# apache/datafusion

Measured on AMD Instinct MI355X. Metric: tpch_q3_hash_join_rows_per_sec, higher is better.
Workload: dtype int64 keys / decimal128 payload; 1 GPU; INNER hash-join orders⋈lineitem on o_orderkey, TPC-H SF100, Q3 payload (o_orderdate,o_shippriority,l_orderkey,l_extendedprice,l_discount), device-resident inputs; build_rows=150000000, probe_rows=599960064, output_rows=599960064, join_table=rank_map, probe=single_pass_unordered, parallelism=single GPU, exchange=none

## Files before the change

datafusion_amd/csrc/aggregate.hip:

```cpp
#include <algorithm>
#include <cstdio>
#include <cstdlib>

#include "device.hpp"
#include "internal.hpp"
#include "rowprog_host.hpp"
#include "grouped.hpp"

namespace dfgpu {

void pack_bytes_to_bitmap(const uint8_t* bytes, int64_t n, uint64_t* words);

constexpr int MAX_AGGS = 16;
constexpr uint32_t PROBE_LIMIT = 256;

enum AccKind : int { ACC_SUM_I64 = 0, ACC_SUM_I128 = 1, ACC_SUM_F64 = 2, ACC_MIN_I64 = 3, ACC_MAX_I64 = 4, ACC_COUNT = 5, ACC_COUNT_STAR = 6,
                     ACC_AND = 7, ACC_OR = 8, ACC_XOR = 9, ACC_KIND_COUNT = 10 };
struct AccKindText {
  const char* type;
  const char* from_u64[2];
  const char* to_u64[2];
  const char* neutral;
  const char* atomic;
  const char* cell_cast;
// ... 1641 lines not shown
      InternCtx sc = ictx;
      sc.slots = sslots->as<uint32_t>();
      sc.mask = 2 * SAMPLE - 1;
      {
        ProfileScope ps("agg_intern_sample", key_bytes / total * SAMPLE);
        k_intern_claim<<<grid_for(SAMPLE, BLOCK), BLOCK, 0, r.stream>>>(sc, SAMPLE, flag->as<int>(), nullptr, 0);
        k_count_slots<<<grid_for(2 * SAMPLE, BLOCK), BLOCK, 0, r.stream>>>(sc.slots, (uint64_t)(2 * SAMPLE), (uint32_t)(SAMPLE / 4), cnt->as<unsigned long long>());
        DFGPU_HIP(hipGetLastError());
      }
      unsigned long long c2[2] = {0, 0};
      d2h(c2, cnt->ptr, 16);
      DFGPU_HIP(hipMemsetAsync(flag->ptr, 0, 4, r.stream));
      const double d_all = (double)c2[0], d_early = (double)c2[1];
      const double est = d_all < 1.25 * d_early ? 2.0 * d_all : d_all / (double)SAMPLE * (double)total;
      uint64_t want = 1 << 16;
      while ((double)want < 3.0 * est && want < cap_max) want <<= 1;
      cap = std::max<uint64_t>(cap, want);
    }
  }
  if (cap > cap_max && !direct_n) cap = cap_max;
  while (!direct_n) {
    R.slots = make_zero_buf((cap + 1) * 4);
    ictx.slots = R.slots->as<uint32_t>();
    ictx.mask = cap - 1;
    if (keyed) {
      R.keyed = make_buf((cap + 1) * sizeof(KeyedSlot));
      ictx.keyed = R.keyed->as<KeyedSlot>();
      k_keyed_clear<<<grid_for((int64_t)cap + 1, BLOCK), BLOCK, 0, r.stream>>>(ictx.keyed, cap + 1);
    }
    if (total) {
      ProfileScope ps(keyed ? "agg_intern_claim_keyed" : "agg_intern_claim", key_bytes);
      if (want_row_slots && !R.row_slot) R.row_slot = make_buf((size_t)total * 4);
      uint32_t* rs = R.row_slot ? R.row_slot->as<uint32_t>() : nullptr;
      if (keyed) {
        k_intern_claim_keyed<<<grid_for((total + KEYED_ROWS - 1) / KEYED_ROWS, BLOCK), BLOCK, 0, r.stream>>>(ictx, total, flag->as<int>(), row_mask, G0, rs);
        k_keyed_rows<<<grid_for((int64_t)cap + 1, BLOCK), BLOCK, 0, r.stream>>>(ictx.keyed, cap + 1, ictx.slots);
      }
      else k_intern_claim<<<grid_for(total, BLOCK), BLOCK, 0, r.stream>>>(ictx, total, flag->as<int>(), row_mask, G0, rs);
      DFGPU_HIP(hipGetLastError());
    }
    int ovf = 0;
    d2h(&ovf, flag->ptr, 4);
    if (!ovf) break;
    DFGPU_CHECK(cap < cap_max, "group table overflow at maximum capacity");
    cap = std::min<uint64_t>(cap_max, cap * 16);
    DFGPU_HIP(hipMemsetAsync(flag->ptr, 0, 4, r.stream));
  }
  A.capacity_hint = (int64_t)cap;
  const int64_t n_words = (total + 63) / 64;
  BufPtr rep_mask = make_zero_buf((size_t)(n_words ? n_words : 1) * 8);
  BufPtr prefix = make_buf((size_t)(n_words + 1) * 8);
  const uint64_t n_slots = cap + (keyed ? 1 : 0);
  k_mark_reps<<<grid_for((int64_t)n_slots, BLOCK), BLOCK, 0, r.stream>>>(R.slots->as<uint32_t>(), n_slots, rep_mask->as<unsigned long long>());
  scan_mask_popcounts(rep_mask->as<uint64_t>(), nullptr, total, prefix->as<uint64_t>());
  R.G1 = (int64_t)read_u64(prefix->as<uint64_t>() + n_words);
  R.slot_gid = make_buf((cap + 1) * 4);
  BufPtr rep_row = make_buf((size_t)(R.G1 ? R.G1 : 1) * 8);
  k_slot_gids<<<grid_for((int64_t)n_slots, BLOCK), BLOCK, 0, r.stream>>>(R.slots->as<uint32_t>(), n_slots, rep_mask->as<uint64_t>(), prefix->as<uint64_t>(),
                                                                      R.slot_gid->as<uint32_t>(), rep_row->as<int64_t>());
  DFGPU_HIP(hipGetLastError());
  Table gk;
  gk.nrows = R.G1;
  for (int g = 0; g < ngk; g++) gk.cols.push_back(gather_column(R.cat_keys[g], rep_row->as<int64_t>(), R.G1, false));
  A.group_keys = std::move(gk);
  return R;
}

__global__ __launch_bounds__(BLOCK) void k_split128(const unsigned long long* __restrict__ cells, int64_t n, unsigned long long* __restrict__ lo, unsigned long long* __restrict__ hi) {
  for (int64_t i = (int64_t)blockIdx.x * BLOCK + threadIdx.x; i < n; i += (int64_t)gridDim.x * BLOCK) {
    lo[i] = cells[2 * i];
    hi[i] = cells[2 * i + 1];
  }
}
static void materialize_seen(Aggregate& A, int64_t G) {
  for (AggState& a : A.aggs) {
    if (!a.seen_all) continue;
    if (G > 0 && a.seen) DFGPU_HIP(hipMemsetD32Async((hipDeviceptr_t)a.seen->ptr, 1, (size_t)G, rt().stream));
    a.seen_all = false;
  }
}
static void split_interleaved(Aggregate& A, int64_t G) {
  materialize_seen(A, G);
  for (AggState& a : A.aggs) {
    if (!a.inter) continue;
    if (G > 0) {
      k_split128<<<grid_for(G, BLOCK), BLOCK, 0, rt().stream>>>(a.inter->as<unsigned long long>(), G, a.lo->as<unsigned long long>(), a.hi->as<unsigned long long>());
      DFGPU_HIP(hipGetLastError());
    }
    a.inter.reset();
  }
}

constexpr int FM_MAX = 4 * MAX_AGGS;
struct FillMany {
  void* p[FM_MAX];
  unsigned long long v[FM_MAX];
  int elem[FM_MAX];
};
__global__ __launch_bounds__(BLOCK) void k_fill_many(FillMany f, int64_t n) {
  const int c = blockIdx.y;
  for (int64_t i = (int64_t)blockIdx.x * BLOCK + threadIdx.x; i < n; i += (int64_t)gridDim.x * BLOCK) {
    if (f.elem[c] == 8) reinterpret_cast<unsigned long long*>(f.p[c])[i] = f.v[c];
    else reinterpret_cast<uint32_t*>(f.p[c])[i] = (uint32_t)f.v[c];
  }
}
static std::vector<AccPlan> grow_accumulators(Aggregate& A, int64_t G0, int64_t G1, bool init = true) {
  std::vector<AccPlan> plans;
  const bool final_mode = A.final_mode();
// ... 1451 lines not shown
        hmm[0] = cached->min;
        hmm[1] = cached->max;
        range_known = true;
      }
    }
  }
  if (range_known) {
    hflags[0] = 0;
    hflags[1] = 1;
  } else {
    {
      ProfileScope ps("agg_dense_key_range", key_bytes);
      jit_launch(f_minmax, grid, BLOCK, 0, &args, sizeof(args));
    }
    d2h(hmm, mm->ptr, 16);
    d2h(hflags, flags->ptr, 8);
  }
  const bool any_rows = hflags[1] != 0, null_group = hflags[0] != 0;
  uint64_t range = any_rows ? (uint64_t)hmm[1] - (uint64_t)hmm[0] + 1 : 0;
  if (range > (1ull << 36) || range > (uint64_t)n * 64) return false;
  fix_argument_types(A, cp, arg_out);
  const int64_t n_words = (int64_t)((range + 63) / 64) + 1;
  BufPtr bits = make_zero_buf((size_t)n_words * 8);
  BufPtr prefix = make_buf((size_t)(n_words + 1) * 8);
  args.bits = bits->as<unsigned long long>();
  args.kmin = any_rows ? hmm[0] : 0;
  const int ncw = (int)cell_kind.size();
  PartValues pv;
  pv.want_rep_mask = option_on("agg.gather_emit", true);
  const bool by_parts = any_rows && !null_group && dense_accumulate_partitioned(A, in, pred, accs, acc_col, acc_val, acc_agg, ncw, args.kmin, range, pv);
  auto dense_emit_of = [&]() {
    DenseEmit e{};
    for (const Ent& en : entries) {
      AggState& a = A.aggs[(size_t)en.agg];
      if (en.is_avg_count) {
        e.dst[e.n_dst] = a.cnt->as<unsigned long long>();
        e.src_word[e.n_dst++] = en.cell;
      } else {
        e.dst[e.n_dst] = a.lo->as<unsigned long long>();
        e.src_word[e.n_dst++] = en.cell;
        if (en.kind == ACC_SUM_I128) {
          e.dst[e.n_dst] = a.hi->as<unsigned long long>();
          e.src_word[e.n_dst++] = en.cell + 1;
        }
        e.seen_dst[e.n_seen] = a.seen->as<uint32_t>();
        e.seen_bit[e.n_seen++] = en.seen_bit;
      }
    }
    return e;
  };
  if (by_parts && pv.rep_mask) {
    const int64_t row_words = (n + 63) / 64;
    BufPtr rprefix = make_buf((size_t)(row_words + 1) * 8);
    scan_mask_popcounts(pv.rep_mask->as<uint64_t>(), nullptr, n, rprefix->as<uint64_t>());
    const int64_t G = (int64_t)read_u64(rprefix->as<uint64_t>() + row_words);
    grow_accumulators(A, 0, G, false);
    const DenseEmit e = dense_emit_of();
    int kci = -1;
    DFGPU_CHECK(is_plain_column(A.group_nodes[0], A.group_roots[0], &kci) && kci >= 0 && kci < (int)in.cols.size(), "internal: the partitioned node's key is not a column");
    const Column& kin = in.cols[(size_t)kci];
    Column kc = alloc_column(kf, A.group_names[0], G);
    kc.dict = kin.dict;
    if (G) {
      ProfileScope ps("agg_dense_gather_emit", n * type_width(kf.type) + G * (type_width(kf.type) + 16 * (int64_t)e.n_dst + 4 * (int64_t)e.n_seen));
      const int g = (int)std::min<int64_t>((row_words + GE_TILE_WORDS - 1) / GE_TILE_WORDS, 2048);
      const uint64_t* rm = pv.rep_mask->as<uint64_t>();
      const uint64_t* rp = rprefix->as<uint64_t>();
      const unsigned long long* cv = pv.cells_v->as<unsigned long long>();
      switch (type_width(kf.type)) {
        case 8: k_dense_gather_emit<int64_t><<<g, BLOCK, 0, r.stream>>>(rm, rp, row_words, (const int64_t*)kin.ptr(), args.kmin, cv, std::max(1, ncw), e, (int64_t*)kc.data->ptr); break;
        case 1: k_dense_gather_emit<uint8_t><<<g, BLOCK, 0, r.stream>>>(rm, rp, row_words, (const uint8_t*)kin.ptr(), args.kmin, cv, std::max(1, ncw), e, (uint8_t*)kc.data->ptr); break;
        default:
          if (kf.type == DFGPU_UINT32) k_dense_gather_emit<uint32_t><<<g, BLOCK, 0, r.stream>>>(rm, rp, row_words, (const uint32_t*)kin.ptr(), args.kmin, cv, std::max(1, ncw), e, (uint32_t*)kc.data->ptr);
          else k_dense_gather_emit<int32_t><<<g, BLOCK, 0, r.stream>>>(rm, rp, row_words, (const int32_t*)kin.ptr(), args.kmin, cv, std::max(1, ncw), e, (int32_t*)kc.data->ptr);
          break;
      }
      DFGPU_HIP(hipGetLastError());
    }
    Table gk;
    gk.nrows = G;
    gk.cols.push_back(std::move(kc));
    A.group_keys = std::move(gk);
    A.ngroups = G;
    DFGPU_HIP(hipStreamSynchronize(r.stream));
    return true;
  }
  if (by_parts) {
    k_presence_bits<<<grid_for(n_words, BLOCK / WAVE), BLOCK, 0, r.stream>>>(pv.first_row_v->as<uint32_t>(), range, n_words, bits->as<uint64_t>());
    DFGPU_HIP(hipGetLastError());
  } else if (any_rows) {
    ProfileScope ps("agg_dense_setbits", key_bytes);
    jit_launch(f_setbits, grid, BLOCK, 0, &args, sizeof(args));
  }
  scan_mask_popcounts(bits->as<uint64_t>(), nullptr, n_words * 64, prefix->as<uint64_t>());
  const int64_t Gk = (int64_t)read_u64(prefix->as<uint64_t>() + n_words);
  const int64_t G = Gk + (null_group ? 1 : 0);
  BufPtr first_row = make_buf((size_t)std::max<int64_t>(G, 1) * 4);
  BufPtr seen = by_parts ? make_buf((size_t)std::max<int64_t>(G, 1) * 4) : make_zero_buf((size_t)std::max<int64_t>(G, 1) * 4);
  BufPtr cells = make_buf((size_t)std::max(1, ncw) * std::max<int64_t>(G, 1) * 8);
  args.prefix = prefix->as<uint64_t>();
  args.first_row = first_row->as<uint32_t>();
  args.cells = cells->as<unsigned long long>();
  args.seen = seen->as<uint32_t>();
  args.G = G;
  args.null_group = null_group ? Gk : -1;
  if (by_parts) {
    if (G) {
      ProfileScope ps("agg_dense_values_to_groups", (int64_t)range * (4 + 8 * ncw) + G * (8 + 8 * ncw));
      k_values_to_groups<<<grid_for((int64_t)range, BLOCK), BLOCK, 0, r.stream>>>(bits->as<uint64_t>(), prefix->as<uint64_t>(), pv.first_row_v->as<uint32_t>(),
                                                                                 pv.cells_v->as<unsigned long long>(), pv.vstride, range, ncw, G, first_row->as<uint32_t>(),
                                                                                 cells->as<unsigned long long>(), seen->as<uint32_t>(), (uint32_t)((1ull << accs.size()) - 1ull));
      DFGPU_HIP(hipGetLastError());
    }
  } else {
    DFGPU_HIP(hipMemsetAsync(first_row->ptr, 0xFF, (size_t)std::max<int64_t>(G, 1) * 4, r.stream));
    for (int w = 0; w < ncw && G; w++)
      k_fill_u64<<<grid_for(G, BLOCK), BLOCK, 0, r.stream>>>(acc_identity(cell_kind[(size_t)w]), G, cells->as<unsigned long long>() + (int64_t)w * G);
    if (G) {
      ProfileScope ps("agg_dense_accumulate", n * cp.input_bytes_per_row);
      jit_launch(f_acc, grid, BLOCK, 0, &args, sizeof(args));
    }
  }
  const int64_t row_words = (n + 63) / 64;
  BufPtr rep_mask = make_zero_buf((size_t)row_words * 8);
  BufPtr rprefix = make_buf((size_t)(row_words + 1) * 8);
  if (G) k_mark_first_rows<<<grid_for(G, BLOCK), BLOCK, 0, r.stream>>>(first_row->as<uint32_t>(), G, rep_mask->as<unsigned long long>());
  scan_mask_popcounts(rep_mask->as<uint64_t>(), nullptr, n, rprefix->as<uint64_t>());
  DFGPU_CHECK((int64_t)read_u64(rprefix->as<uint64_t>() + row_words) == G, "dense-key node: first-row marks do not match the group count");
  grow_accumulators(A, 0, G, false);
  const DenseEmit e = dense_emit_of();
  BufPtr new_gid = make_buf((size_t)std::max<int64_t>(G, 1) * 4);
  BufPtr key_i64 = make_zero_buf((size_t)std::max<int64_t>(G, 1) * 8);
  if (G) {
    ProfileScope ps("agg_dense_emit", G * (4 + 8 * (int64_t)e.n_dst));
    k_dense_permute<<<grid_for(G, BLOCK), BLOCK, 0, r.stream>>>(first_row->as<uint32_t>(), cells->as<unsigned long long>(), seen->as<uint32_t>(), G,
                                                                rep_mask->as<uint64_t>(), rprefix->as<uint64_t>(), new_gid->as<uint32_t>(), e);
    k_dense_keys<<<grid_for(n_words, BLOCK / WAVE), BLOCK, 0, r.stream>>>(bits->as<uint64_t>(), prefix->as<uint64_t>(), n_words, args.kmin, new_gid->as<uint32_t>(),
                                                                          key_i64->as<unsigned long long>());
    DFGPU_HIP(hipGetLastError());
  }
  Column kc = alloc_column(kf, A.group_names[0], G);
  {
    int key_col = -1;
    if (is_plain_column(A.group_nodes[0], A.group_roots[0], &key_col) && key_col >= 0 && key_col < (int)in.cols.size()) kc.dict = in.cols[key_col].dict;
  }
  if (G) {
    int mode = 0;
    if (kf.type == DFGPU_INT32 || kf.type == DFGPU_DATE32 || kf.type == DFGPU_UINT32) mode = 3;
    else if (kf.type == DFGPU_UINT8) mode = 4;
    k_emit_values<<<grid_for(G, BLOCK), BLOCK, 0, r.stream>>>(mode, key_i64->as<unsigned long long>(), nullptr, nullptr, G, kc.data->ptr, nullptr);
    DFGPU_HIP(hipGetLastError());
    if (null_group) {
      uint32_t ng = 0;
      d2h(&ng, new_gid->as<uint32_t>() + Gk, 4);
      std::vector<uint8_t> vb((size_t)G, 1);
      vb[ng] = 0;
      BufPtr dvb = make_buf((size_t)G + 64);
      h2d_async(dvb->ptr, vb.data(), (size_t)G);
      kc.validity = make_buf(bitmap_bytes(G));
      pack_bytes_to_bitmap(dvb->as<uint8_t>(), G, kc.validity->as<uint64_t>());
      kc.null_count = 1;
      DFGPU_HIP(hipStreamSynchronize(r.stream));
    }
  }
  Table gk;
  gk.nrows = G;
  gk.cols.push_back(std::move(kc));
  A.group_keys = std::move(gk);
  A.ngroups = G;
  DFGPU_HIP(hipStreamSynchronize(r.stream));
  return true;
}

template <typename T>
__global__ __launch_bounds__(BLOCK) void k_run_heads(const T* __restrict__ key, int64_t n, uint64_t* __restrict__ heads) {
  const int64_t n_words = (n + 63) >> 6;
  const int64_t wave = ((int64_t)blockIdx.x * BLOCK + threadIdx.x) >> 6;
  const int64_t n_waves = ((int64_t)gridDim.x * BLOCK) >> 6;
  const unsigned lane = lane_id();
  constexpr int U = 4;
  for (int64_t w0 = wave * U; w0 < n_words; w0 += n_waves * U) {
// ... 248 lines not shown
  src += "  }\n}\n";
  return src + args_size_check(sizeof(RunsNodeArgs), "RunsNodeArgs");
}

static bool agg_update_sorted_runs_jit(Aggregate& A, const Table& in, const dfgpu_expr* pred) {
  Runtime& r = rt();
  const int64_t n = in.nrows;
  if (pred || !option_on("jit", true) || !option_on("agg.runs", true) || A.group_roots.empty() || A.ngroups != 0) return false;
  if (n < option_int("jit.min_rows", policy().rows_worth_a_pass()) || n >= 0xFFFFFFFFll) return false;
  int key_col = -1;
  if (!is_plain_column(A.group_nodes[0], A.group_roots[0], &key_col) || key_col < 0 || key_col >= (int)in.cols.size()) return false;
  const Column& kcol = in.cols[(size_t)key_col];
  const dfgpu_field kf = kcol.field;
  if (kcol.validity || !(kf.type == DFGPU_INT32 || kf.type == DFGPU_INT64 || kf.type == DFGPU_DATE32 || kf.type == DFGPU_UINT32 || kf.type == DFGPU_UINT8)) return false;
  std::vector<int> more_keys;
  for (size_t g = 1; g < A.group_roots.size(); g++) {
    int c = -1;
    if (!is_plain_column(A.group_nodes[g], A.group_roots[g], &c) || c < 0 || c >= (int)in.cols.size()) return false;
    const Column& mc = in.cols[(size_t)c];
    if (mc.validity || mc.field.type == DFGPU_BOOL || mc.field.type == DFGPU_UTF8) return false;
    more_keys.push_back(c);
  }
  if (!column_stats(const_cast<Column&>(kcol), n).nondecreasing) return false;
  std::string why;
  RowProgramCompiler comp(in);
  dfgpu_expr ke{A.group_nodes[0].data(), (int)A.group_nodes[0].size(), A.group_roots[0]};
  const int key_out = comp.add_output(ke);
  const std::vector<int> arg_out = compile_agg_arguments(comp, A);
  CompiledProgram cp;
  if (!comp.finish(cp, why)) return false;
  const std::vector<AccEntry> entries = accumulator_entries(A, cp, arg_out);
  std::vector<RunsAcc> accs;
  for (const AccEntry& en : entries) {
    const dfgpu_field& t = en.type;
    accs.push_back({en.kind, en.val, en.kind == ACC_SUM_I128 && t.type == DFGPU_DECIMAL128 && t.precision > 0 && t.precision <= 16,
                    en.kind == ACC_SUM_I128 && A.aggs[(size_t)en.agg].func == DFGPU_AGG_SUM && t.type == DFGPU_DECIMAL128});
  }
  if (accs.size() > (size_t)RUNS_MAX_ACCS) return false;
  const std::string source = agg_runs_node_source(cp, cp.src_out_vals[(size_t)key_out], kf.type, accs);
  hipFunction_t f_acc = nullptr;
  if (!jit_get_kernels(source, {{"runs_accumulate", &f_acc}})) return false;
  const int64_t n_words = (n + 63) / 64;
  BufPtr heads = make_buf((size_t)n_words * 8);
  {
    ProfileScope ps("agg_runs_heads", n * type_width(kf.type));
    const int g = grid_for(n_words, (BLOCK / WAVE) * 4);
    switch (type_width(kf.type)) {
      case 8: k_run_heads<uint64_t><<<g, BLOCK, 0, r.stream>>>((const uint64_t*)kcol.ptr(), n, heads->as<uint64_t>()); break;
      case 4: k_run_heads<uint32_t><<<g, BLOCK, 0, r.stream>>>((const uint32_t*)kcol.ptr(), n, heads->as<uint64_t>()); break;
      default: k_run_heads<uint8_t><<<g, BLOCK, 0, r.stream>>>((const uint8_t*)kcol.ptr(), n, heads->as<uint64_t>()); break;
    }
    DFGPU_HIP(hipGetLastError());
  }
  BufPtr prefix = make_buf((size_t)(n_words + 1) * 8);
  scan_mask_popcounts(heads->as<uint64_t>(), nullptr, n, prefix->as<uint64_t>());
  BufPtr long_flag = make_zero_buf(8);
  k_run_long_flag<<<grid_for(n_words, BLOCK), BLOCK, 0, r.stream>>>(heads->as<uint64_t>(), n_words, long_flag->as<uint32_t>());
  if (!more_keys.empty()) {
    int64_t bytes = 0;
    for (int c : more_keys) bytes += n * type_width(in.cols[(size_t)c].field.type);
    ProfileScope ps("agg_runs_dependent_keys", bytes);
    const int g = grid_for(n, BLOCK * 4);
    for (int c : more_keys) {
      const Column& mc = in.cols[(size_t)c];
      uint32_t* fl = long_flag->as<uint32_t>() + 1;
      switch (type_width(mc.field.type)) {
        case 16: k_run_dependent<uint4><<<g, BLOCK, 0, r.stream>>>((const uint4*)mc.ptr(), heads->as<uint64_t>(), n, fl); break;
        case 8: k_run_dependent<uint64_t><<<g, BLOCK, 0, r.stream>>>((const uint64_t*)mc.ptr(), heads->as<uint64_t>(), n, fl); break;
        case 4: k_run_dependent<uint32_t><<<g, BLOCK, 0, r.stream>>>((const uint32_t*)mc.ptr(), heads->as<uint64_t>(), n, fl); break;
        default: k_run_dependent<uint8_t><<<g, BLOCK, 0, r.stream>>>((const uint8_t*)mc.ptr(), heads->as<uint64_t>(), n, fl); break;
      }
    }
    DFGPU_HIP(hipGetLastError());
  }
  const int64_t G = (int64_t)read_u64(prefix->as<uint64_t>() + n_words);
  uint32_t flags[2] = {0, 0};
  d2h(flags, long_flag->ptr, 8);
  if (flags[1]) return false;
  const uint32_t has_long = flags[0];
  fix_argument_types(A, cp, arg_out);
  grow_accumulators(A, 0, G, has_long != 0);
  Column kc = alloc_like(kcol, G);
  kc.name = A.group_names[0];
  RunsNodeArgs args{};
  set_input_columns(args, cp);
  args.heads = heads->as<uint64_t>();
  args.prefix = prefix->as<uint64_t>();
  args.key_out = kc.data->ptr;
  args.n = n;
  for (size_t e = 0; e < entries.size(); e++) {
    AggState& a = A.aggs[(size_t)entries[e].agg];
    if (entries[e].is_avg_count) {
      args.cell[2 * e] = a.cnt->as<unsigned long long>();
    } else if (accs[e].inter) {
      a.inter = has_long ? make_zero_buf((size_t)(G ? G : 1) * 16) : make_buf((size_t)(G ? G : 1) * 16);
      args.cell[2 * e] = a.inter->as<unsigned long long>();
      args.cell[2 * e + 1] = a.inter->as<unsigned long long>() + 1;
      args.seen[e] = a.seen->as<uint32_t>();
    } else {
      args.cell[2 * e] = a.lo->as<unsigned long long>();
      if (entries[e].kind == ACC_SUM_I128) args.cell[2 * e + 1] = a.hi->as<unsigned long long>();
      args.seen[e] = a.seen->as<uint32_t>();
    }
    if (!entries[e].is_avg_count && accs[e].val >= 0 && !cp.src_maybe_null[(size_t)accs[e].val] && option_on("agg.runs_seen_all", true)) {
      args.seen[e] = nullptr;
      a.seen_all = true;
    }
  }
  {
    ProfileScope ps("agg_runs_accumulate", n * cp.input_bytes_per_row);
    const int max_blocks = (int)option_int("agg.runs_max_blocks", 1 << 30);
    jit_launch(f_acc, std::max(1, std::min(grid_for(n_words, BLOCK / WAVE), max_blocks)), BLOCK, 0, &args, sizeof(args));
  }
  Table gk;
  gk.nrows = G;
  gk.cols.push_back(std::move(kc));
  if (!more_keys.empty()) {
    Table heads_rows = compact_table(in, more_keys, heads->as<uint64_t>(), nullptr);
    for (size_t g = 0; g < more_keys.size(); g++) {
      heads_rows.cols[g].name = A.group_names[g + 1];
      gk.cols.push_back(std::move(heads_rows.cols[g]));
    }
  }
  A.group_keys = std::move(gk);
  A.ngroups = G;
  DFGPU_HIP(hipStreamSynchronize(r.stream));
  return true;
}

__global__ __launch_bounds__(BLOCK) void k_small_reset(SmallAccSet accs, int D, uint32_t* __restrict__ g_first, uint32_t* __restrict__ g_seen) {
// ... 1038 lines not shown
```

datafusion_amd/csrc/device.hpp:

```cpp
#pragma once
#include <hip/hip_runtime.h>
#include <stdint.h>

namespace dfgpu {

typedef __int128 i128;
typedef unsigned __int128 u128;

constexpr int WAVE = 64;
constexpr int BLOCK = 256;

__device__ __forceinline__ unsigned lane_id() { return threadIdx.x & 63u; }

#ifndef DFGPU_STREAM_NT
#define DFGPU_STREAM_NT 3
#endif
template <typename T>
__device__ __forceinline__ T stream_load(const T* p) {
#if DFGPU_STREAM_NT & 1
  return __builtin_nontemporal_load(p);
#else
  return *p;
#endif
}
// ... 156 lines not shown
__device__ __forceinline__ bool keys_equal(const KeySet& a, int64_t ia, const KeySet& b, int64_t ib, bool null_equals_null) {
  for (int c = 0; c < a.n; c++) {
    bool va = !a.c[c].valid || bit_at(a.c[c].valid, ia);
    bool vb = !b.c[c].valid || bit_at(b.c[c].valid, ib);
    if (!va || !vb) {
      if (null_equals_null && !va && !vb) continue;
      return false;
    }
    uint64_t alo, ahi, blo, bhi;
    load_words(a.c[c], ia, alo, ahi);
    load_words(b.c[c], ib, blo, bhi);
    if (alo != blo || ahi != bhi) return false;
  }
  return true;
}

__host__ __device__ __forceinline__ int32_t date32_part(int32_t days, int part) {
  const int64_t z = (int64_t)days + 719468;
  const int64_t era = (z >= 0 ? z : z - 146096) / 146097;
  const int64_t doe = z - era * 146097;
  const int64_t yoe = (doe - doe / 1460 + doe / 36524 - doe / 146096) / 365;
  const int64_t doy = doe - (365 * yoe + yoe / 4 - yoe / 100);
  const int64_t mp = (5 * doy + 2) / 153;
  const int64_t d = doy - (153 * mp + 2) / 5 + 1;
  const int64_t m = mp < 10 ? mp + 3 : mp - 9;
  const int64_t y = yoe + era * 400 + (m <= 2 ? 1 : 0);
  return (int32_t)(part == 0 ? y : part == 1 ? m : d);
}

struct FastMod {
  uint64_t M;
  uint32_t n, c;
};
inline FastMod fastmod_for(uint32_t n) { return FastMod{~0ull / n + 1ull, n, (uint32_t)((1ull << 32) % n)}; }
__host__ __device__ __forceinline__ uint32_t fastmod_u32(uint32_t x, const FastMod& f) {
#if defined(__HIP_DEVICE_COMPILE__)
  return (uint32_t)__umul64hi(f.M * x, (uint64_t)f.n);
#else
  return (uint32_t)(((unsigned __int128)(f.M * x) * f.n) >> 64);
#endif
}
__host__ __device__ __forceinline__ uint32_t fastmod_u64(uint64_t h, const FastMod& f) {
  if ((f.n & (f.n - 1)) == 0) return (uint32_t)h & (f.n - 1);
  const uint32_t a = fastmod_u32((uint32_t)(h >> 32), f), b = fastmod_u32((uint32_t)h, f);
  return fastmod_u32(a * f.c + b, f);
}

inline int grid_for(int64_t work_items, int per_block) {
  int64_t b = (work_items + per_block - 1) / per_block;
  if (b < 1) b = 1;
  if (b > 256 * 8) b = 256 * 8;
  return (int)b;
}

constexpr uint64_t TS_AGG = 1ull << 62, TS_PFX = 2ull << 62, TS_VAL = (1ull << 62) - 1;

__device__ __forceinline__ uint64_t ts_load(const uint64_t* p) { return __hip_atomic_load(p, __ATOMIC_RELAXED, __HIP_MEMORY_SCOPE_AGENT); }
__device__ __forceinline__ void ts_store(uint64_t* p, uint64_t v) { __hip_atomic_store(p, v, __ATOMIC_RELAXED, __HIP_MEMORY_SCOPE_AGENT); }

__device__ __forceinline__ uint64_t lookback_exclusive(uint64_t* __restrict__ tile_state, int64_t tile, uint64_t agg) {
  const unsigned lane = lane_id();
  uint64_t excl = 0;
  if (tile > 0) {
    if (lane == 0) ts_store(&tile_state[tile], TS_AGG | agg);
    constexpr int LB = 4;
    int64_t base = tile - 1;
    for (;;) {
      uint64_t sum, pfx_lanes;
      for (;;) {
        uint64_t st[LB];
#pragma unroll
        for (int q = 0; q < LB; q++) {
          const int64_t idx = base - ((int64_t)lane * LB + q);
          st[q] = idx >= 0 ? ts_load(&tile_state[idx]) : TS_PFX;
        }
        sum = 0;
        bool lane_pfx = false, lane_block = false;
#pragma unroll
        for (int q = 0; q < LB; q++) {
          const unsigned status = (unsigned)(st[q] >> 62);
          if (!lane_pfx && !lane_block) {
            if (status == 0) lane_block = true;
            else {
              sum += st[q] & TS_VAL;
              lane_pfx = status == 2;
            }
          }
        }
        pfx_lanes = ballot64(lane_pfx);
        const uint64_t block_lanes = ballot64(lane_block);
        const int first_pfx = pfx_lanes ? __builtin_ctzll(pfx_lanes) : 64;
        const int first_block = block_lanes ? __builtin_ctzll(block_lanes) : 64;
        if (first_block > first_pfx || !block_lanes) break;
        __builtin_amdgcn_s_sleep(1);
      }
      const int first_pfx = pfx_lanes ? __builtin_ctzll(pfx_lanes) : 64;
      excl += wave_sum((int)lane <= first_pfx ? sum : 0ull);
      if (first_pfx < 64) break;
      base -= 64 * LB;
    }
  }
  if (lane == 0) ts_store(&tile_state[tile], TS_PFX | (excl + agg));
  return excl;
}

}
// ... 1 lines not shown
```

datafusion_amd/csrc/filter.hip:

```cpp
#include <algorithm>
#include <cstdlib>

#include "device.hpp"
#include "internal.hpp"
#include "records.hpp"

namespace dfgpu {

constexpr int MAX_COLS = 12;
struct CopyCols {
  const void* src[MAX_COLS];
  void* dst[MAX_COLS];
  const uint64_t* src_valid[MAX_COLS];
  uint8_t* dst_valid_bytes[MAX_COLS];
  int width[MAX_COLS];
  int n;
};

template <typename T>
__device__ __forceinline__ void copy_elem(const void* src, void* dst, int64_t s, int64_t d) {
  reinterpret_cast<T*>(dst)[d] = reinterpret_cast<const T*>(src)[s];
}
__device__ __forceinline__ void copy_by_width(int width, const void* src, void* dst, int64_t s, int64_t d) {
  switch (width) {
// ... 73 lines not shown
  }
}

__global__ __launch_bounds__(BLOCK) void k_count_bits(const uint64_t* __restrict__ words, int64_t nrows, unsigned long long* out) {
  const int64_t n_words = (nrows + 63) >> 6;
  uint64_t s = 0;
  for (int64_t w = (int64_t)blockIdx.x * BLOCK + threadIdx.x; w < n_words; w += (int64_t)gridDim.x * BLOCK) {
    uint64_t m = words[w];
    int64_t rem = nrows - (w << 6);
    if (rem < 64) m &= (~0ull) >> (64 - rem);
    s += __popcll(m);
  }
  s = wave_sum(s);
  __shared__ unsigned long long s_part[BLOCK / WAVE];
  if (lane_id() == 0) s_part[threadIdx.x >> 6] = s;
  __syncthreads();
  if (threadIdx.x == 0) {
    unsigned long long t = 0;
#pragma unroll
    for (int w = 0; w < BLOCK / WAVE; w++) t += s_part[w];
    if (t) atomicAdd(out, t);
  }
}

void pack_bytes_to_bitmap(const uint8_t* bytes, int64_t n, uint64_t* words) {
  if (n == 0) return;
  ProfileScope ps("pack_bytes", n + n / 8);
  k_pack_bytes<<<grid_for((n + 63) / 64, BLOCK / WAVE), BLOCK, 0, rt().stream>>>(bytes, n, words);
}

void count_nulls(Column& c) {
  if (!c.validity) {
    c.null_count = 0;
    return;
  }
  if (c.length == 0) {
    c.null_count = 0;
    c.validity.reset();
    return;
  }
  BufPtr cnt = make_zero_buf(8);
  k_count_bits<<<grid_for((c.length + 63) / 64, BLOCK), BLOCK, 0, rt().stream>>>(c.valid_words(), c.length, cnt->as<unsigned long long>());
  uint64_t valid = read_u64(cnt->as<uint64_t>());
  c.null_count = c.length - (int64_t)valid;
  if (c.null_count == 0) c.validity.reset();
}

Table compact_table(const Table& in, const std::vector<int>& cols, const uint64_t* mask, const uint64_t* mask_valid) {
  Runtime& r = rt();
  const int64_t n = in.nrows;
  const int64_t n_words = (n + 63) / 64;
  Table out;
  BufPtr prefix = make_buf((size_t)(n_words + 1) * 8);
  scan_mask_popcounts(mask, mask_valid, n, prefix->as<uint64_t>());
  const int64_t n_out = (int64_t)read_u64(prefix->as<uint64_t>() + n_words);
  out.nrows = n_out;
  std::vector<BufPtr> valid_bytes(cols.size());
  for (size_t i = 0; i < cols.size(); i++) {
    DFGPU_CHECK(cols[i] >= 0 && cols[i] < (int)in.cols.size(), "projection index out of range");
    const Column& c = in.cols[cols[i]];
    if (c.field.type == DFGPU_UTF8) {
      out.cols.push_back(compact_strings(c, mask, mask_valid, prefix->as<uint64_t>(), n, n_out));
      continue;
    }
    out.cols.push_back(alloc_like(c, n_out));
    if (c.validity) valid_bytes[i] = make_buf((size_t)n_out + 64);
  }
  if (n_out > 0) {
    std::vector<int> wide, bits;
    for (size_t i = 0; i < cols.size(); i++) {
      if (in.cols[cols[i]].field.type == DFGPU_UTF8) continue;
      (in.cols[cols[i]].field.type == DFGPU_BOOL ? bits : wide).push_back((int)i);
    }
    for (int i : bits) {
      const Column& c = in.cols[cols[i]];
      BufPtr vals = make_buf((size_t)n_out + 64);
      k_compact_bits<<<grid_for(n_words, BLOCK / WAVE), BLOCK, 0, r.stream>>>((const uint64_t*)c.ptr(), c.valid_words(), mask, mask_valid, prefix->as<uint64_t>(), n,
                                                                               vals->as<uint8_t>(), valid_bytes[i] ? valid_bytes[i]->as<uint8_t>() : nullptr);
      DFGPU_HIP(hipGetLastError());
      pack_bytes_to_bitmap(vals->as<uint8_t>(), n_out, out.cols[i].data->as<uint64_t>());
    }
    for (size_t c0 = 0; c0 < wide.size(); c0 += MAX_COLS) {
      CopyCols cc{};
      int64_t bytes = 0;
      cc.n = (int)std::min<size_t>(MAX_COLS, wide.size() - c0);
      for (int k = 0; k < cc.n; k++) {
        const Column& c = in.cols[cols[wide[c0 + k]]];
        cc.src[k] = c.ptr();
        cc.dst[k] = out.cols[wide[c0 + k]].data->ptr;
        cc.width[k] = type_width(c.field.type);
        cc.src_valid[k] = c.valid_words();
        cc.dst_valid_bytes[k] = valid_bytes[wide[c0 + k]] ? valid_bytes[wide[c0 + k]]->as<uint8_t>() : nullptr;
        bytes += (n + n_out) * cc.width[k];
      }
      ProfileScope ps("compact", bytes + n / 8);
      k_compact<<<grid_for(n_words, (BLOCK / WAVE) * COMPACT_UNROLL), BLOCK, 0, r.stream>>>(cc, mask, mask_valid, prefix->as<uint64_t>(), n);
      DFGPU_HIP(hipGetLastError());
    }
    for (size_t i = 0; i < cols.size(); i++) {
      if (!valid_bytes[i]) continue;
      Column& oc = out.cols[i];
      oc.validity = make_buf(bitmap_bytes(n_out));
      pack_bytes_to_bitmap(valid_bytes[i]->as<uint8_t>(), n_out, oc.validity->as<uint64_t>());
      oc.null_count = -1;
    }
  }
  return out;
}
// ... 293 lines not shown
```

datafusion_amd/csrc/internal.hpp:

```cpp
#pragma once
#include <atomic>
#include <hip/hip_runtime.h>

#include <chrono>
#include <cstdint>
#include <cstring>
#include <map>
#include <memory>
#include <mutex>
#include <stdexcept>
#include <string>
#include <thread>
#include <vector>

#include "../../include/dfgpu.h"

namespace dfgpu {

struct Error : std::runtime_error {
  using std::runtime_error::runtime_error;
};

void set_last_error(const std::string& msg);

// ... 97 lines not shown
int64_t scan_upload_caches_bytes(int device);
Runtime& rt_of(int device);
void use_device(int device);
int current_device();
const std::vector<int>& initialised_devices();
void require_init();

struct ProfileScope {
  hipEvent_t a = nullptr, b = nullptr;
  const char* name;
  int64_t bytes;
  ProfileScope(const char* name, int64_t algorithmic_bytes);
  ~ProfileScope();
};
struct LateRecord {
  hipEvent_t a = nullptr, b = nullptr;
  LateRecord();
  ~LateRecord();
  LateRecord(const LateRecord&) = delete;
  LateRecord& operator=(const LateRecord&) = delete;
  void stop();
  void record(const char* name, int64_t algorithmic_bytes);
  static void label(const char* name);
};

struct DevBuf {
  void* ptr = nullptr;
  size_t bytes = 0;
  Runtime* owner = nullptr;
  std::shared_ptr<void> foreign;
  std::atomic<uint64_t> hint{0};
  std::atomic<uint64_t> all_hit_hint{0};
  explicit DevBuf(size_t n);
  DevBuf(void* p, size_t n, std::shared_ptr<void> keep_alive) : ptr(p), bytes(n), foreign(std::move(keep_alive)) {}
  ~DevBuf();
  DevBuf(const DevBuf&) = delete;
  DevBuf& operator=(const DevBuf&) = delete;
  template <typename T>
  T* as() const { return reinterpret_cast<T*>(ptr); }
};
using BufPtr = std::shared_ptr<DevBuf>;
inline BufPtr make_buf(size_t bytes) { return std::make_shared<DevBuf>(bytes ? bytes : 1); }
BufPtr make_zero_buf(size_t bytes);

void pool_admit(int64_t bytes);
int64_t pool_free_bytes();

void d2h(void* dst, const void* src, size_t n);
struct HostFlag {
  volatile unsigned* host = nullptr;
  unsigned* dev = nullptr;
};
HostFlag* thread_host_flag();
extern std::atomic<int64_t> g_pinned_driver_allocs, g_pinned_driver_ns;
void* pinned_alloc(size_t n);
void pinned_release(void* p);
void* stage_alloc(size_t n);
template <class T> struct StageAllocator {
  using value_type = T;
  StageAllocator() = default;
  template <class U> StageAllocator(const StageAllocator<U>&) {}
  T* allocate(size_t n) { return static_cast<T*>(stage_alloc(n * sizeof(T))); }
  void deallocate(T* p, size_t) { pinned_release(p); }
  template <class U> void construct(U* p) noexcept { ::new ((void*)p) U; }
  template <class U, class... A> void construct(U* p, A&&... a) { ::new ((void*)p) U(std::forward<A>(a)...); }
  template <class U> bool operator==(const StageAllocator<U>&) const { return true; }
  template <class U> bool operator!=(const StageAllocator<U>&) const { return false; }
};
template <class T> using StageVec = std::vector<T, StageAllocator<T>>;
struct PinnedBuf {
  void* ptr = nullptr;
  size_t bytes = 0;
  explicit PinnedBuf(size_t n) : ptr(pinned_alloc(n ? n : 1)), bytes(n) {}
  ~PinnedBuf() { pinned_release(ptr); }
  PinnedBuf(const PinnedBuf&) = delete;
  PinnedBuf& operator=(const PinnedBuf&) = delete;
  template <class T> T* as() const { return reinterpret_cast<T*>(ptr); }
};
void h2d_async(void* dst, const void* src, size_t n);

inline int type_width(int t) {
  switch (t) {
    case DFGPU_INT32: case DFGPU_UINT32: case DFGPU_DATE32: return 4;
    case DFGPU_INT64: case DFGPU_UINT64: case DFGPU_FLOAT64: return 8;
    case DFGPU_DECIMAL128: return 16;
    case DFGPU_UINT8: return 1;
    case DFGPU_BOOL: return 0;
    case DFGPU_UTF8:
      throw Error("a Utf8 column reached an operator that works on fixed-width columns: dictionary-encode it first (dfgpu_table_dictionary_encode)");
  }
  throw Error("unknown dfgpu_type " + std::to_string(t));
}
inline size_t bitmap_bytes(int64_t n) { return (size_t)((n + 63) / 64) * 8; }
inline size_t data_bytes(int t, int64_t n) { return t == DFGPU_BOOL ? bitmap_bytes(n) : (size_t)n * type_width(t); }
inline bool is_integer_like(int t) {
  return t == DFGPU_INT32 || t == DFGPU_INT64 || t == DFGPU_UINT8 || t == DFGPU_UINT32 || t == DFGPU_UINT64 || t == DFGPU_DATE32;
}
inline bool is_signed_type(int t) { return t == DFGPU_INT32 || t == DFGPU_INT64 || t == DFGPU_DATE32 || t == DFGPU_DECIMAL128; }
std::string type_name(const dfgpu_field& f);

struct ColStats {
  long long min = 0, max = 0;
  int64_t valid = 0;
  bool ascending = false;
  bool nondecreasing = false;
  bool has_present = false;
// ... 12 lines not shown
inline bool same_dictionary(const std::shared_ptr<const DictValues>& a, const std::shared_ptr<const DictValues>& b) {
  return a == b || (a && b && a->values == b->values && a->valid == b->valid);
}

struct Column {
  dfgpu_field field{};
  std::string name;
  int64_t length = 0;
  int64_t null_count = 0;
  BufPtr data;
  size_t data_offset = 0;
  BufPtr validity;
  BufPtr offsets;
  std::shared_ptr<ColStats> stats;
  std::shared_ptr<const DictValues> dict;

  const void* ptr() const { return data ? (const char*)data->ptr + data_offset : nullptr; }
  const uint64_t* valid_words() const { return validity ? validity->as<uint64_t>() : nullptr; }
  bool has_nulls() const { return validity != nullptr; }
};

struct Table {
  std::vector<Column> cols;
  int64_t nrows = 0;
  int device = current_device();
};

inline Table* unwrap(dfgpu_table_t t) {
  DFGPU_CHECK(t != nullptr, "null table handle");
  Table* p = reinterpret_cast<Table*>(t);
  if (p->device >= 0) use_device(p->device);
  thread_metrics().rows_in += p->nrows;
  return p;
}
inline Table* unwrap_quiet(dfgpu_table_t t) {
  Table* p = unwrap(t);
  thread_metrics().rows_in -= p->nrows;
  return p;
}
inline dfgpu_table_t wrap(Table* t) {
  thread_metrics().rows_out += t->nrows;
  return reinterpret_cast<dfgpu_table_t>(t);
}

Column alloc_column(const dfgpu_field& f, const std::string& name, int64_t n, bool with_validity = false);
inline Column alloc_like(const Column& src, int64_t n, bool with_validity = false) {
  Column c = alloc_column(src.field, src.name, n, with_validity);
  c.dict = src.dict;
  return c;
}

inline dfgpu_table_t wrap_quiet(Table* t) { return reinterpret_cast<dfgpu_table_t>(t); }

void scan_mask_popcounts(const uint64_t* mask, const uint64_t* valid, int64_t nrows, uint64_t* out_prefix);
void scan_u32(const uint32_t* in, int64_t n, uint64_t* out_prefix);
uint64_t read_u64(const uint64_t* dev);

Table compact_table(const Table& in, const std::vector<int>& cols, const uint64_t* mask, const uint64_t* mask_valid);
Column gather_column(const Column& in, const int64_t* idx, int64_t n, bool idx_may_be_null);
std::vector<Column> gather_columns(const Table& in, const std::vector<int>& cols, const int64_t* idx, int64_t n, bool idx_may_be_null, const uint32_t* idx32 = nullptr);
struct PackLayout;
bool plan_record_layout(const Table& in, const std::vector<int>& cols, PackLayout& L, int& R, std::vector<int>& order);
Column bool_as_u8(const Column& c, int64_t n);
void and_bitmaps(const uint64_t* a, const uint64_t* b, int64_t nw, uint64_t* out);
void count_nulls(Column& c);

struct Datum {
  Column col;
  std::string str;
  bool scalar = false;
  bool scalar_null = false;
  uint64_t lit_lo = 0, lit_hi = 0;
};
dfgpu_field expr_type(const dfgpu_expr& e, const Table& input);
Datum evaluate(const dfgpu_expr& e, const Table& input);
Column datum_to_column(const Datum& d, int64_t n, const std::string& name);

inline const int64_t* str_offsets(const Column& c) { return c.offsets ? c.offsets->as<int64_t>() : nullptr; }
Column alloc_string_column(const Column& like, int64_t n);
Column gather_strings(const Column& in, const int64_t* idx, int64_t n, bool idx_may_be_null);
Column substr_column(const Column& in, int64_t start, bool has_count, int64_t count);
Column compact_strings(const Column& in, const uint64_t* mask, const uint64_t* mask_valid, const uint64_t* prefix, int64_t nrows, int64_t n_out);
Column slice_strings(const Column& in, int64_t offset, int64_t length);
Column concat_strings(const std::vector<const Column*>& parts, int64_t total);
Column dictionary_encode(const Column& in, bool sorted);
Column dictionary_decode(const Column& in);
Column string_hash_column(const Column& in);
Datum string_binary(int op, const Datum& a, const Datum& b, int64_t nrows);

hipFunction_t jit_get(const std::string& source, const char* kernel_name);
void jit_launch(hipFunction_t fn, int grid, int block, size_t lds_bytes, void* args, size_t args_bytes);

dfgpu_field parse_format(const char* fmt, bool nullable);
std::string format_of(const dfgpu_field& f);
int64_t table_device_bytes(const Table& t);

Column remap_to_dictionary(const Column& c, const std::shared_ptr<const DictValues>& target);
Column dictionary_like_column(const Column& c, const std::string& pattern, bool case_insensitive);

void bitmap_place(const uint64_t* src, int64_t off, int64_t n, uint64_t* dst);

ColStats column_stats(Column& c, int64_t nrows);

std::vector<uint8_t> join_visited_export(dfgpu_join_t h);
void join_visited_merge(dfgpu_join_t h, const uint8_t* merged, size_t nbytes);

void join_bytes_mask(const uint8_t* bytes, int64_t n, bool want_set, uint64_t* mask);
void join_append_unmatched(const uint64_t* mask, const uint64_t* prefix, int64_t n, int64_t base, int64_t* null_side, int64_t* row_side);
// ... 30 lines not shown
```

datafusion_amd/csrc/join.hip:

```cpp
#include <thread>
#include <functional>
#include <cstdlib>

#include "device.hpp"
#include "internal.hpp"
#include "grouped.hpp"

namespace dfgpu {

Table compact_table(const Table& in, const std::vector<int>& cols, const uint64_t* mask, const uint64_t* mask_valid);
void pack_bytes_to_bitmap(const uint8_t* bytes, int64_t n, uint64_t* words);

enum TableKind : int { KIND_HASH = 0, KIND_ARRAY = 1, KIND_RANK = 2, KIND_RADIX = 3, KIND_FLAT = 4, KIND_FLAT16 = 5,
                       KIND_RETURNED = 6 };
template <int KIND> constexpr bool kind_is_flat() { return KIND == KIND_FLAT || KIND == KIND_FLAT16; }
template <int KIND> constexpr bool kind_is_direct() { return KIND == KIND_ARRAY || KIND == KIND_RANK; }

struct FlatLayout {
  int n;
  uint8_t off[MAX_KEYS];
  uint8_t width[MAX_KEYS];
  int8_t null_bit[MAX_KEYS];
};
constexpr double RANK_MAP_MIN_KEY_DENSITY = 1.0 / 256.0;
// ... 86 lines not shown
#pragma unroll
    for (int j = 0; j < W; j++) {
      const int64_t p = ((w0 + j) << 6) + lane;
      u[j] = NT ? __builtin_nontemporal_load(d + (p < np ? p : np - 1)) : d[p < np ? p : np - 1];
    }
    const long long keep = q.is_unsigned[i] ? 0xFFFFFFFFll : -1ll;
#pragma unroll
    for (int j = 0; j < W; j++) v[j] = (long long)(int32_t)u[j] & keep;
  } else {
    const uint8_t* d = reinterpret_cast<const uint8_t*>(q.data[i]);
#pragma unroll
    for (int j = 0; j < W; j++) {
      const int64_t p = ((w0 + j) << 6) + lane;
      v[j] = (long long)(NT ? __builtin_nontemporal_load(d + (p < np ? p : np - 1)) : d[p < np ? p : np - 1]);
    }
  }
}
__device__ __forceinline__ bool rowpred_cmp(unsigned sel, long long v, long long lit) {
  return ((v < lit ? sel : v == lit ? sel >> 1 : sel >> 2) & 1u) != 0;
}
static unsigned rowpred_sel(int op) {
  switch (op) {
    case DFGPU_EXPR_EQ: return 2u;
    case DFGPU_EXPR_NE: return 5u;
    case DFGPU_EXPR_LT: return 1u;
    case DFGPU_EXPR_LE: return 3u;
    case DFGPU_EXPR_GT: return 4u;
    default: return 6u;
  }
}

static KeySet make_keyset(const Table& t, const std::vector<int>& cols) {
  KeySet ks{};
  DFGPU_CHECK((int)cols.size() <= MAX_KEYS, "too many join key columns");
  ks.n = (int)cols.size();
  for (int i = 0; i < ks.n; i++) {
    DFGPU_CHECK(cols[i] >= 0 && cols[i] < (int)t.cols.size(), "join key column index out of range");
    const Column& c = t.cols[cols[i]];
    DFGPU_CHECK(c.field.type != DFGPU_BOOL, "Boolean join keys are not supported on the GPU path");
    ks.c[i] = KeyCol{c.ptr(), c.valid_words(), c.field.type, type_width(c.field.type)};
  }
  return ks;
}


struct MinMax {
  long long smin, smax;
  unsigned long long valid;
  unsigned unsorted;
  unsigned descends;
};
constexpr int BUILD_UNROLL = 4;
template <int KT, bool HASV>
__global__ __launch_bounds__(BLOCK) void k_key_minmax(KeyCol k, int64_t n, MinMax* out) {
  long long mn = INT64_MAX, mx = INT64_MIN;
  unsigned long long cnt = 0;
  bool unsorted = false, descends = false;
  const int64_t stride = (int64_t)gridDim.x * BLOCK;
  for (int64_t i0 = (int64_t)blockIdx.x * BLOCK + threadIdx.x; i0 < n; i0 += stride * BUILD_UNROLL) {
    uint64_t lo[BUILD_UNROLL], plo[BUILD_UNROLL];
    bool ok[BUILD_UNROLL], pok[BUILD_UNROLL];
#pragma unroll
    for (int j = 0; j < BUILD_UNROLL; j++) {
      int64_t i = i0 + j * stride;
      int64_t ic = i < n ? i : n - 1;
      lo[j] = load_key<KT>(k, ic);
      plo[j] = load_key<KT>(k, ic > 0 ? ic - 1 : 0);
    }
#pragma unroll
    for (int j = 0; j < BUILD_UNROLL; j++) {
      int64_t i = i0 + j * stride;
      ok[j] = i < n;
      pok[j] = i < n && i > 0;
      if (HASV) {
        ok[j] = ok[j] && bit_at(k.valid, i < n ? i : n - 1);
        pok[j] = pok[j] && bit_at(k.valid, (i < n ? i : n - 1) > 0 ? (i < n ? i : n - 1) - 1 : 0);
      }
    }
#pragma unroll
    for (int j = 0; j < BUILD_UNROLL; j++) {
      int64_t i = i0 + j * stride;
      if (i < n && !ok[j]) unsorted = descends = true;
      if (!ok[j]) continue;
      long long v = (long long)lo[j];
      mn = v < mn ? v : mn;
      mx = v > mx ? v : mx;
      cnt++;
      if (pok[j] && (long long)plo[j] >= v) unsorted = true;
      if (pok[j] && (long long)plo[j] > v) descends = true;
    }
  }
#pragma unroll
  for (int d = 32; d >= 1; d >>= 1) {
    long long omn = __shfl_xor(mn, d, 64), omx = __shfl_xor(mx, d, 64);
    mn = omn < mn ? omn : mn;
    mx = omx > mx ? omx : mx;
    cnt += __shfl_xor(cnt, d, 64);
  }
  const unsigned wave_unsorted = (ballot64(unsorted) != 0 ? 1u : 0u) | (ballot64(descends) != 0 ? 2u : 0u);
  __shared__ long long s_mn[BLOCK / WAVE], s_mx[BLOCK / WAVE];
  __shared__ unsigned long long s_cnt[BLOCK / WAVE];
  __shared__ unsigned s_uns[BLOCK / WAVE];
  const int wv = threadIdx.x >> 6;
  if (lane_id() == 0) { s_mn[wv] = mn; s_mx[wv] = mx; s_cnt[wv] = cnt; s_uns[wv] = wave_unsorted; }
  __syncthreads();
  if (threadIdx.x == 0) {
    unsigned uns = 0;
    for (int i = 1; i < BLOCK / WAVE; i++) {
      mn = s_mn[i] < mn ? s_mn[i] : mn;
      mx = s_mx[i] > mx ? s_mx[i] : mx;
      cnt += s_cnt[i];
    }
    for (int i = 0; i < BLOCK / WAVE; i++) uns |= s_uns[i];
    if (cnt) {
      atomicMin(&out->smin, mn);
      atomicMax(&out->smax, mx);
      atomicAdd(&out->valid, cnt);
    }
    if (uns & 1u) atomicOr(&out->unsorted, 1u);
    if (uns & 2u) atomicOr(&out->descends, 1u);
  }
}

template <int KT>
__global__ void k_key_ends(KeyCol k, int64_t n, int64_t every, int samples, long long* __restrict__ out) {
  const int i = blockIdx.x * blockDim.x + threadIdx.x;
  if (i == 0) {
    out[0] = (long long)load_key<KT>(k, 0);
    out[1] = (long long)load_key<KT>(k, n - 1);
  }
  if (i >= samples) return;
  const int64_t r = (int64_t)i * every;
  if (r + 1 >= n) return;
  if ((long long)load_key<KT>(k, r + 1) <= (long long)load_key<KT>(k, r)) atomicOr((unsigned long long*)&out[2], 1ull);
}

template <int KT, bool HASV, bool ASCENDING, bool VERIFY = false>
__global__ __launch_bounds__(BLOCK) void k_rank_setbits(KeyCol k, int64_t n, uint64_t offset, unsigned long long* __restrict__ bits, int* dup_flag, uint64_t range = 0) {
  if (ASCENDING) {
    const unsigned lane = lane_id();
    const int64_t stride = (int64_t)gridDim.x * BLOCK;
    for (int64_t base = (int64_t)blockIdx.x * BLOCK + (threadIdx.x & ~63u); base < n; base += stride * BUILD_UNROLL) {
      uint64_t idx[BUILD_UNROLL], pidx[BUILD_UNROLL];
#pragma unroll
      for (int j = 0; j < BUILD_UNROLL; j++) {
        int64_t i = base + j * stride + lane;
        idx[j] = load_key<KT, true>(k, i < n ? i : n - 1) - offset;
        if (VERIFY) pidx[j] = load_key<KT>(k, i < n ? (i > 0 ? i - 1 : 0) : n - 1) - offset;
      }
#pragma unroll
      for (int j = 0; j < BUILD_UNROLL; j++) {
        const int64_t i = base + j * stride + lane;
        bool ok = i < n;
        if (VERIFY) {
          const bool bad = ok && (idx[j] > range || (i > 0 && idx[j] <= pidx[j]));
          if (ballot64(bad) != 0 && lane == 0) atomicOr(dup_flag, 1);
          ok = ok && idx[j] <= range;
        }
        const uint64_t w = ok ? (idx[j] >> 6) : ~0ull;
        const uint64_t v = ok ? 1ull << (idx[j] & 63) : 0ull;
        const uint64_t inc = wave_inclusive_sum_dpp(v);
        const uint64_t w_next = __shfl_down(w, 1, 64);
        const uint64_t tails = ballot64(lane == 63 || w_next != w);
        const uint64_t heads = (tails << 1) | 1ull;
        const int head_lane = 63 - __builtin_clzll(heads & ((2ull << lane) - 1ull));
        const uint64_t before = __shfl(inc - v, head_lane, 64);
        if (ok && ((tails >> lane) & 1ull)) atomicOr(&bits[w], (unsigned long long)(inc - before));
      }
    }
    return;
  }
  const int64_t stride = (int64_t)gridDim.x * BLOCK;
  for (int64_t i0 = (int64_t)blockIdx.x * BLOCK + threadIdx.x; i0 < n; i0 += stride * BUILD_UNROLL) {
    uint64_t lo[BUILD_UNROLL];
    bool ok[BUILD_UNROLL];
#pragma unroll
    for (int j = 0; j < BUILD_UNROLL; j++) {
      int64_t i = i0 + j * stride;
      lo[j] = load_key<KT>(k, i < n ? i : n - 1);
    }
#pragma unroll
    for (int j = 0; j < BUILD_UNROLL; j++) {
      int64_t i = i0 + j * stride;
      ok[j] = i < n;
      if (HASV) ok[j] = ok[j] && bit_at(k.valid, i < n ? i : n - 1);
    }
#pragma unroll
// ... 1460 lines not shown
    const int64_t p = (w << 6) + lane_id();
    const bool hit = p < np && hits[p] != 0;
    if (bytes && p < np) bytes[p] = hit ? 1 : 0;
    const uint64_t word = ballot64(p < np && (hit == (want != 0)));
    if (lane_id() == 0) mask[w] = word;
  }
}
__global__ __launch_bounds__(BLOCK) void k_append_unmatched(const uint64_t* __restrict__ mask, const uint64_t* __restrict__ prefix, int64_t np, int64_t base,
                                                           int64_t* __restrict__ ob2, int64_t* __restrict__ op2) {
  const int64_t n_words = (np + 63) >> 6;
  const int64_t wave = ((int64_t)blockIdx.x * BLOCK + threadIdx.x) >> 6;
  const int64_t n_waves = ((int64_t)gridDim.x * BLOCK) >> 6;
  for (int64_t w = wave; w < n_words; w += n_waves) {
    const uint64_t mk = mask[w];
    if ((mk >> lane_id()) & 1ull) {
      const int64_t d = base + (int64_t)(prefix[w] + mbcnt(mk));
      ob2[d] = -1;
      op2[d] = (w << 6) + lane_id();
    }
  }
}

__global__ __launch_bounds__(BLOCK) void k_visited_mask(const uint8_t* __restrict__ visited, int64_t n, int want_visited, uint64_t* __restrict__ mask) {
  const int64_t n_words = (n + 63) >> 6;
  const int64_t wave = ((int64_t)blockIdx.x * BLOCK + threadIdx.x) >> 6;
  const int64_t n_waves = ((int64_t)gridDim.x * BLOCK) >> 6;
  for (int64_t w = wave; w < n_words; w += n_waves) {
    int64_t i = (w << 6) + lane_id();
    uint64_t word = ballot64(i < n && ((visited[i] != 0) == (want_visited != 0)));
    if (lane_id() == 0) mask[w] = word;
  }
}

template <typename F>
static void with_kind(int kind, F&& f) {
  switch (kind) {
    case KIND_ARRAY: f(std::integral_constant<int, KIND_ARRAY>{}); break;
    case KIND_RANK: f(std::integral_constant<int, KIND_RANK>{}); break;
    case KIND_FLAT: f(std::integral_constant<int, KIND_FLAT>{}); break;
    case KIND_FLAT16: f(std::integral_constant<int, KIND_FLAT16>{}); break;
    default: f(std::integral_constant<int, KIND_HASH>{}); break;
  }
}
template <typename F>
static void with_key_type(int dfgpu_type, F&& f) {
  switch (dfgpu_type) {
    case DFGPU_INT32: case DFGPU_DATE32: f(std::integral_constant<int, KT_I32>{}); break;
    case DFGPU_UINT32: f(std::integral_constant<int, KT_U32>{}); break;
    case DFGPU_INT64: f(std::integral_constant<int, KT_I64>{}); break;
    case DFGPU_UINT8: f(std::integral_constant<int, KT_U8>{}); break;
    default: throw Error("key type has no direct-address instantiation");
  }
}
template <typename F>
static void with_kind_and_key(int kind, int probe_key_type, F&& f) {
  if (kind == KIND_HASH) {
    f(std::integral_constant<int, KIND_HASH>{}, std::integral_constant<int, KT_ANY>{});
    return;
  }
  if (kind == KIND_FLAT) {
    f(std::integral_constant<int, KIND_FLAT>{}, std::integral_constant<int, KT_ANY>{});
    return;
  }
  if (kind == KIND_FLAT16) {
    f(std::integral_constant<int, KIND_FLAT16>{}, std::integral_constant<int, KT_ANY>{});
    return;
  }
  if (kind == KIND_RETURNED) {
    f(std::integral_constant<int, KIND_RETURNED>{}, std::integral_constant<int, KT_ANY>{});
    return;
  }
  with_key_type(probe_key_type, [&](auto kt) {
    if (kind == KIND_ARRAY) f(std::integral_constant<int, KIND_ARRAY>{}, kt);
    else f(std::integral_constant<int, KIND_RANK>{}, kt);
  });
}

static void ensure_rank_tab(JoinTable& jt) {
  if (jt.kind != KIND_RANK) return;
  std::lock_guard<std::mutex> lk(jt.tab_mu);
  if (jt.rank_tab) return;
  DFGPU_CHECK(jt.rank_bits && jt.rank_prefix, "internal: rank map without a table and without bitmap + prefix");
  Runtime& r = rt();
  const int64_t n_words = (int64_t)((jt.am_size - 1) >> 6) + 1;
  BufPtr tab = make_buf((size_t)n_words * 16);
  {
    ProfileScope ps("join_build_rank_interleave", n_words * 16);
    k_rank_interleave<<<grid_for(n_words, BLOCK), BLOCK, 0, r.stream>>>(jt.rank_bits->as<uint64_t>(), jt.rank_prefix->as<uint64_t>(), n_words, tab->as<ulonglong2>());
    DFGPU_HIP(hipGetLastError());
  }
  call_epilogue();
  jt.rank_tab = tab;
  std::lock_guard<std::mutex> lk2(jt.mu);
  jt.info.table_bytes += n_words * 16;
}

static void ensure_rank_bits(JoinTable& jt) {
  if (jt.kind != KIND_RANK) return;
  std::lock_guard<std::mutex> lk(jt.tab_mu);
  if (jt.rank_bits) return;
  DFGPU_CHECK(jt.rank_tab != nullptr, "internal: rank map without a table and without bitmap + prefix");
  Runtime& r = rt();
  const int64_t n_words = (int64_t)((jt.am_size - 1) >> 6) + 1;
  BufPtr bits = make_buf((size_t)n_words * 8);
  {
    ProfileScope ps("join_build_rank_deinterleave", n_words * 24);
// ... 123 lines not shown
                                                        bool speculate) {
  Runtime& r = rt();
  auto jt = std::make_unique<JoinTable>();
  jt->build = build;
  jt->key_cols = key_cols;
  jt->null_equality = null_equality;
  jt->force_collisions = opts.force_hash_collisions != 0;
  jt->probe_mode = opts.probe_mode;
  jt->null_aware = opts.null_aware != 0;
  if (jt->null_aware) {
    DFGPU_CHECK(key_cols.size() == 1,
                "null_aware anti join only supports single column join key, got " + std::to_string(key_cols.size()) + " columns");
    DFGPU_CHECK(key_cols[0] >= 0 && key_cols[0] < (int)build.cols.size(), "build key column out of range");
    jt->build_side_has_null = null_count_of(build.cols[key_cols[0]]) > 0;
  }
  const int64_t nb = build.nrows;
  DFGPU_CHECK(nb < 0xFFFFFFFFll, "build side has >= u32::MAX rows (the reference switches to JoinHashMapU64; not supported on GPU)");
  KeySet ks = make_keyset(build, key_cols);
  jt->info.build_rows = nb;

  if (opts.table_mode == 4) {
    jt->kind = KIND_RADIX;
    jt->radix = radix_join_build(build, key_cols, null_equality == DFGPU_NULL_EQUALS_NULL, jt->force_collisions);
    jt->keys_unique = false;
    jt->info.table_bytes = radix_join_table_bytes(*jt->radix);
    jt->info.table_kind = KIND_RADIX;
    jt->info.build_keys_unique = 0;
    return jt;
  }
  bool have_stats = false, ascending = false;
  uint64_t range = 0;
  long long kmin = 0;
  int64_t n_valid_keys = 0;
  bool speculated = false;
  const bool spec_off = false;
  std::shared_ptr<ColStats> known;
  if (ks.n == 1 && opts.table_mode != 1 && opts.table_mode != 5 && is_integer_like(ks.c[0].type) && ks.c[0].type != DFGPU_UINT64 && option_on("join.cached_key_stats", true)) {
    const Column& kc = build.cols[key_cols[0]];
    known = std::atomic_load(&kc.stats);
    const bool null_block = null_equality == DFGPU_NULL_EQUALS_NULL && kc.has_nulls();
    if (known && !null_block && nb > 0 && known->valid > 0) {
      range = (uint64_t)known->max - (uint64_t)known->min;
      have_stats = range != UINT64_MAX;
      kmin = known->min;
      ascending = known->ascending;
      n_valid_keys = known->valid;
    } else {
      known.reset();
    }
  }
  if (!known && speculate && !spec_off && (opts.table_mode == 0 || opts.table_mode == 3) && ks.n == 1 && is_integer_like(ks.c[0].type) && ks.c[0].type != DFGPU_UINT64 &&
      !ks.c[0].valid && nb >= (1 << 22)) {
    constexpr int S = 4096;
    BufPtr ends = make_zero_buf(24);
    with_key_type(ks.c[0].type, [&](auto kt) { k_key_ends<decltype(kt)::value><<<S / BLOCK, BLOCK, 0, r.stream>>>(ks.c[0], nb, nb / S, S, ends->as<long long>()); });
    long long e[3] = {0, 0, 1};
    d2h(e, ends->ptr, 24);
    const uint64_t grange = (uint64_t)e[1] - (uint64_t)e[0];
    if (e[2] == 0 && e[1] > e[0] && grange != UINT64_MAX && grange + 1 >= (uint64_t)nb && grange < (1ull << 40)) {
      const double gdense = (double)nb / ((double)grange + 1.0);
      if (grange < (uint64_t)opts.perfect_hash_join_small_build_threshold || gdense >= RANK_MAP_MIN_KEY_DENSITY || opts.table_mode == 3) {
        speculated = true;
        have_stats = true;
        ascending = true;
        range = grange;
        kmin = e[0];
        n_valid_keys = nb;
      }
    }
  }
  if (!known && !speculated && opts.table_mode != 1 && opts.table_mode != 5 && ks.n == 1 && is_integer_like(ks.c[0].type) && ks.c[0].type != DFGPU_UINT64) {
    const Column& kc = build.cols[key_cols[0]];
    bool null_block = null_equality == DFGPU_NULL_EQUALS_NULL && kc.has_nulls();
    if (!null_block && nb > 0) {
      BufPtr mm = make_buf(sizeof(MinMax));
      static const MinMax init{INT64_MAX, INT64_MIN, 0, 0, 0};
      h2d_async(mm->ptr, &init, sizeof init);
      {
        ProfileScope ps("join_build_key_stats", nb * ks.c[0].width);
        const int g = std::min(grid_for(nb, BLOCK * BUILD_UNROLL), 512);
        with_key_type(ks.c[0].type, [&](auto kt) {
          constexpr int T = decltype(kt)::value;
          if (ks.c[0].valid) k_key_minmax<T, true><<<g, BLOCK, 0, r.stream>>>(ks.c[0], nb, mm->as<MinMax>());
          else k_key_minmax<T, false><<<g, BLOCK, 0, r.stream>>>(ks.c[0], nb, mm->as<MinMax>());
        });
      }
      MinMax res;
      d2h(&res, mm->ptr, sizeof res);
      n_valid_keys = (int64_t)res.valid;
      if (res.valid > 0) {
        range = (uint64_t)res.smax - (uint64_t)res.smin;
        have_stats = range != UINT64_MAX;
        kmin = res.smin;
        ascending = res.unsorted == 0;
        std::atomic_store(&const_cast<Column&>(kc).stats, std::make_shared<ColStats>(ColStats{res.smin, res.smax, (int64_t)res.valid, res.unsorted == 0, res.descends == 0}));
      }
    }
  }
  const double dense = have_stats ? (double)nb / ((double)range + 1.0) : 0.0;
  bool am_ok = have_stats && !(range >= (uint64_t)opts.perfect_hash_join_small_build_threshold && dense <= opts.perfect_hash_join_min_key_density);
  if (opts.table_mode == 2) am_ok = have_stats;
  am_ok = am_ok && range < (1ull << 34);
  bool rank_ok = have_stats && (opts.table_mode == 0 || opts.table_mode == 3) && range < (1ull << 40) &&
                 (range < (uint64_t)opts.perfect_hash_join_small_build_threshold || dense >= RANK_MAP_MIN_KEY_DENSITY || opts.table_mode == 3);
  DFGPU_CHECK(!speculated || rank_ok, "internal: speculative build statistics outside the rank map's gate");
  DFGPU_CHECK(!(opts.table_mode == 2 && !am_ok), "direct-address join table requested but not applicable");
  DFGPU_CHECK(!(opts.table_mode == 3 && !rank_ok), "rank-map join table requested but not applicable");
  constexpr int64_t MALL_BYTES = (int64_t)256 << 20;

  BufPtr flag;
  auto need_flag = [&]() {
    if (!flag) flag = make_zero_buf(4);
    return flag->as<int>();
  };
  int dup = 0;
  bool flat_wide = false;
  if (rank_ok && !ascending && !speculated && opts.table_mode == 0 && opts.probe_mode == 4 && ks.n == 1 && nb * 8 > MALL_BYTES && nb >= ((int64_t)1 << 22)) {
    const int64_t m = (int64_t)1 << 18;
    const uint64_t slots = (uint64_t)1 << 20;
    BufPtr table = make_zero_buf((size_t)slots * 8);
    {
      ProfileScope ps("join_build_sample_duplicates", m * 2 * ks.c[0].width);
      with_key_type(ks.c[0].type, [&](auto kt) {
        k_sample_duplicates<decltype(kt)::value><<<grid_for(2 * m, BLOCK), BLOCK, 0, r.stream>>>(ks.c[0], nb, nb / m, m, table->as<unsigned long long>(), slots - 1, need_flag());
      });
      DFGPU_HIP(hipGetLastError());
    }
    int seen = 0;
    d2h(&seen, need_flag(), 4);
    if (seen) {
      dup = 1;
      rank_ok = false;
      DFGPU_HIP(hipMemsetAsync(need_flag(), 0, 4, r.stream));
    }
  }
  if (rank_ok) {
    const int64_t n_words = (int64_t)(range >> 6) + 1;
    BufPtr eager_tab;
    if (ascending && (double)nb >= 0.15 * ((double)range + 1.0)) {
      const bool no_fill = known && known->ascending && known->valid == nb && known->onepass_fit == (RT_FIT_TAG | 1ull) && option_on("join.onepass_no_fill", true);
      eager_tab = no_fill ? make_buf((size_t)n_words * 16) : make_zero_buf((size_t)n_words * 16);
      ProfileScope ps("join_build_rank_tab_onepass", nb * ks.c[0].width + n_words * 16);
      const int g = (int)((nb + RT_ROWS - 1) / RT_ROWS);
      with_key_type(ks.c[0].type, [&](auto kt) {
        constexpr int T = decltype(kt)::value;
        if (speculated) k_rank_tab_onepass<T, true><<<g, BLOCK, 0, r.stream>>>(ks.c[0], nb, (uint64_t)kmin, range, eager_tab->as<ulonglong2>(), need_flag());
        else if (no_fill) k_rank_tab_onepass<T, false, true><<<g, BLOCK, 0, r.stream>>>(ks.c[0], nb, (uint64_t)kmin, range, eager_tab->as<ulonglong2>(), nullptr);
        else k_rank_tab_onepass<T, false><<<g, BLOCK, 0, r.stream>>>(ks.c[0], nb, (uint64_t)kmin, range, eager_tab->as<ulonglong2>(), nullptr);
      });
      if (no_fill && r.profiling) {
        std::lock_guard<std::mutex> lk(r.mu);
        r.recs.push_back(Runtime::Rec{"join_build_rank_tab_no_fill", nullptr, nullptr, 0, std::this_thread::get_id()});
      }
      DFGPU_HIP(hipGetLastError());
    } else {
    jt->rank_bits = make_zero_buf((size_t)n_words * 8);
    {
      ProfileScope ps("join_build_rank_map", nb * ks.c[0].width);
      int g = std::min(grid_for(nb, BLOCK * BUILD_UNROLL), 2048);
      unsigned long long* bits = jt->rank_bits->as<unsigned long long>();
      KeyCol kc0 = ks.c[0];
      BufPtr grouped_keys;
      constexpr int RB_BITS = 10;
      const bool lds_bits = !ascending && nb > (1 << 22) && n_words * 8 > ((int64_t)16 << 20) && (range >> RB_BITS) < (1ull << 20) - 64;
      if (lds_bits) {
        const GroupSpec gs = group_spec((uint64_t)kmin, range + 1, 1 << RB_BITS);
        GroupedRows gr = group_rows_by_key(kc0, nb, gs, RB_BITS, nullptr, true, false, {}, {}, "join_build_group_keys");
        const int P = 1 << RB_BITS;
        std::vector<uint64_t> gfirst((size_t)P + 1);
        uint64_t max_span = 0;
        for (int q = 0; q <= P; q++) {
          const unsigned __int128 v = ((((unsigned __int128)(unsigned)q) << 64) + gs.mul - 1) / gs.mul;
          gfirst[(size_t)q] = v > (unsigned __int128)(range + 1) || q == P ? range + 1 : (uint64_t)v;
          if (q) max_span = std::max(max_span, gfirst[(size_t)q] - gfirst[(size_t)q - 1]);
        }
        BufPtr d_first = make_buf(gfirst.size() * 8);
        h2d_async(d_first->ptr, gfirst.data(), gfirst.size() * 8);
        const size_t lds = (size_t)((max_span >> 6) + 2) * 8;
        DFGPU_HIP(hipFuncSetAttribute(reinterpret_cast<const void*>(k_rank_bits_grouped), hipFuncAttributeMaxDynamicSharedMemorySize, (int)lds));
        k_rank_bits_grouped<<<P, RB_THREADS, lds, r.stream>>>(gr.keys->as<uint64_t>(), gr.bounds->as<uint64_t>(), d_first->as<uint64_t>(), (uint64_t)kmin, bits, need_flag());
        DFGPU_HIP(hipGetLastError());
        DFGPU_HIP(hipStreamSynchronize(r.stream));
      } else {
      if (!ascending && !kc0.valid && kc0.width == 8 && nb > (1 << 22) && n_words * 8 > ((int64_t)16 << 20)) {
        const Column& kcol = build.cols[(size_t)key_cols[0]];
        grouped_keys = kcol.data;
        if (kcol.data_offset != 0) {
          grouped_keys = make_buf((size_t)nb * 8);
          DFGPU_HIP(hipMemcpyAsync(grouped_keys->ptr, kcol.ptr(), (size_t)nb * 8, hipMemcpyDeviceToDevice, r.stream));
        }
        int range_bits = 0;
        while (range_bits < 64 && ((range + 1) >> range_bits)) range_bits++;
        radix_group_keys(grouped_keys, nb, std::max(0, range_bits - 6), 6);
        kc0.data = grouped_keys->ptr;
      }
      const bool byte_map = !ascending && nb > (1 << 20) && range < (1ull << 32);
      if (byte_map) {
        BufPtr bytes = make_zero_buf((size_t)n_words * 64);
        with_key_type(kc0.type, [&](auto kt) {
          constexpr int T = decltype(kt)::value;
          if (kc0.valid) k_rank_setbytes<T, true><<<g, BLOCK, 0, r.stream>>>(kc0, nb, (uint64_t)kmin, bytes->as<uint8_t>());
          else k_rank_setbytes<T, false><<<g, BLOCK, 0, r.stream>>>(kc0, nb, (uint64_t)kmin, bytes->as<uint8_t>());
        });
        DFGPU_HIP(hipGetLastError());
        pack_bytes_to_bitmap(bytes->as<uint8_t>(), n_words * 64, jt->rank_bits->as<uint64_t>());
      } else {
      with_key_type(kc0.type, [&](auto kt) {
        constexpr int T = decltype(kt)::value;
        if (speculated) k_rank_setbits<T, false, true, true><<<g, BLOCK, 0, r.stream>>>(kc0, nb, (uint64_t)kmin, bits, need_flag(), range);
        else if (ascending) k_rank_setbits<T, false, true><<<g, BLOCK, 0, r.stream>>>(kc0, nb, (uint64_t)kmin, bits, need_flag());
        else if (kc0.valid) k_rank_setbits<T, true, false><<<g, BLOCK, 0, r.stream>>>(kc0, nb, (uint64_t)kmin, bits, need_flag());
        else k_rank_setbits<T, false, false><<<g, BLOCK, 0, r.stream>>>(kc0, nb, (uint64_t)kmin, bits, need_flag());
      });
      }
      }
    }
    jt->rank_prefix = make_buf((size_t)(n_words + 1) * 8);
    scan_mask_popcounts(jt->rank_bits->as<uint64_t>(), nullptr, n_words * 64, jt->rank_prefix->as<uint64_t>());
    if (!ascending) dup = (int64_t)read_u64(jt->rank_prefix->as<uint64_t>() + n_words) != n_valid_keys;
    }
    if (speculated) {
      int wrong = 0;
      d2h(&wrong, need_flag(), 4);
      if (wrong & 1) {
        ProfileScope ps("join_build_speculation_missed", 0);
        jt.reset();
        return join_build_fixed_keys(build, key_cols, null_equality, opts, false);
      }
      ColStats st{kmin, (long long)((uint64_t)kmin + range), nb, true, true};
      if (eager_tab) st.onepass_fit = RT_FIT_TAG | ((wrong & 2) ? 0ull : 1ull);
      std::atomic_store(&const_cast<Column&>(build.cols[key_cols[0]]).stats, std::make_shared<ColStats>(st));
    }
    if (!dup) {
      jt->kind = KIND_RANK;
      jt->am_offset = (uint64_t)kmin;
      jt->am_size = range + 1;
      jt->rank_needs_perm = !ascending;
      jt->info.table_bytes = n_words * 16;
      jt->rank_tab = eager_tab;
    } else {
      DFGPU_CHECK(opts.table_mode != 3, "rank-map join table requested but not applicable: the build keys are not unique");
      jt->rank_bits.reset();
      jt->rank_prefix.reset();
    }
  }
  if (opts.table_mode == 0 && dup && opts.probe_mode == 4 && ks.n == 1 && nb * 8 > MALL_BYTES) {
    jt->rank_bits.reset();
    jt->kind = KIND_RADIX;
    jt->radix = radix_join_build(build, key_cols, null_equality == DFGPU_NULL_EQUALS_NULL, jt->force_collisions);
    jt->keys_unique = false;
    jt->info.table_bytes = radix_join_table_bytes(*jt->radix);
    jt->info.table_kind = KIND_RADIX;
    jt->info.build_keys_unique = 0;
    return jt;
  }
  if (jt->kind != KIND_RANK && am_ok) {
    jt->kind = KIND_ARRAY;
    jt->array_map = true;
    jt->am_offset = (uint64_t)kmin;
    jt->am_size = range + 1;
    jt->heads = make_zero_buf(jt->am_size * 4);
    auto am_build = [&](uint32_t* next) {
      const int g = std::min(grid_for(nb, BLOCK * BUILD_UNROLL), 2048);
      with_key_type(ks.c[0].type, [&](auto kt) {
        constexpr int T = decltype(kt)::value;
        if (ks.c[0].valid) k_am_build<T, true><<<g, BLOCK, 0, r.stream>>>(ks.c[0], nb, jt->am_offset, jt->heads->as<uint32_t>(), next, need_flag());
        else k_am_build<T, false><<<g, BLOCK, 0, r.stream>>>(ks.c[0], nb, jt->am_offset, jt->heads->as<uint32_t>(), next, need_flag());
      });
    };
    if (dup) jt->next = make_zero_buf((size_t)nb * 4);
    {
      ProfileScope ps("join_build_array_map", nb * ks.c[0].width);
      am_build(dup ? jt->next->as<uint32_t>() : nullptr);
    }
    if (!dup) {
      d2h(&dup, need_flag(), 4);
// ... 79 lines not shown
  jt->info.build_keys_ascending = ascending;
  return jt;
}

static Table with_build_dictionaries(const JoinTable& jt, const Table& probe, std::vector<int>& pk) {
  DFGPU_CHECK(pk.size() == jt.key_cols.size(), "probe key count differs from build key count");
  Table fixed;
  bool changed = false;
  for (size_t i = 0; i < pk.size(); i++) {
    DFGPU_CHECK(pk[i] >= 0 && pk[i] < (int)probe.cols.size(), "join key column index out of range");
    const Column& bc = jt.build.cols[jt.key_cols[i]];
    if (probe.cols[pk[i]].field.type == DFGPU_BOOL) {
      DFGPU_CHECK(bc.field.type == DFGPU_UINT8 && !bc.dict, "join key types differ between build and probe side (the planner inserts casts)");
      if (!changed) fixed = probe;
      changed = true;
      fixed.cols.push_back(bool_as_u8(probe.cols[pk[i]], probe.nrows));
      pk[i] = (int)fixed.cols.size() - 1;
      continue;
    }
    if (bc.dict && probe.cols[pk[i]].field.type == DFGPU_UTF8 && !probe.cols[pk[i]].dict) {
      Column enc = dictionary_encode(probe.cols[pk[i]], true);
      if (!same_dictionary(bc.dict, enc.dict)) {
        for (size_t k = 0; k < bc.dict->valid.size(); k++) DFGPU_CHECK(bc.dict->valid[k], "join keys with NULL dictionary values and different dictionaries are not supported on the GPU path");
        enc = remap_to_dictionary(enc, bc.dict);
      }
      if (!changed) fixed = probe;
      changed = true;
      fixed.cols.push_back(enc);
      pk[i] = (int)fixed.cols.size() - 1;
      continue;
    }
    const Column& pc = probe.cols[pk[i]];
    DFGPU_CHECK((bc.dict != nullptr) == (pc.dict != nullptr), "join key " + std::to_string(i) + ": one side is dictionary-encoded, the other is not (the planner inserts casts)");
    if (!bc.dict || same_dictionary(bc.dict, pc.dict)) continue;
    for (size_t k = 0; k < bc.dict->valid.size(); k++) DFGPU_CHECK(bc.dict->valid[k], "join keys with NULL dictionary values and different dictionaries are not supported on the GPU path");
    for (size_t k = 0; k < pc.dict->valid.size(); k++) DFGPU_CHECK(pc.dict->valid[k], "join keys with NULL dictionary values and different dictionaries are not supported on the GPU path");
    if (!changed) fixed = probe;
    changed = true;
    fixed.cols[pk[i]] = remap_to_dictionary(pc, bc.dict);
  }
  return changed ? fixed : probe;
}

static JoinTable* unwrap_join(dfgpu_join_t ht) {
  DFGPU_CHECK(ht != nullptr, "null join handle");
  JoinTable* jt = reinterpret_cast<JoinTable*>(ht);
  if (jt->build.device >= 0) use_device(jt->build.device);
  return jt;
}

ColStats column_stats(Column& kc, int64_t nrows) {
  DFGPU_CHECK(is_integer_like(kc.field.type) && kc.field.type != DFGPU_UINT64, "dfgpu_column_minmax: integer columns only");
  if (auto cached = std::atomic_load(&kc.stats)) return *cached;
  Runtime& r = rt();
  MinMax res{INT64_MAX, INT64_MIN, 0, 0, 0};
  if (nrows > 0) {
    KeyCol k{kc.ptr(), kc.valid_words(), kc.field.type, type_width(kc.field.type)};
    BufPtr mm = make_buf(sizeof(MinMax));
    h2d_async(mm->ptr, &res, sizeof res);
    {
      ProfileScope ps("column_minmax", nrows * k.width);
      const int g = std::min(grid_for(nrows, BLOCK * BUILD_UNROLL), 512);
      with_key_type(k.type, [&](auto kt) {
        constexpr int T = decltype(kt)::value;
        if (k.valid) k_key_minmax<T, true><<<g, BLOCK, 0, r.stream>>>(k, nrows, mm->as<MinMax>());
        else k_key_minmax<T, false><<<g, BLOCK, 0, r.stream>>>(k, nrows, mm->as<MinMax>());
      });
      DFGPU_HIP(hipGetLastError());
    }
    d2h(&res, mm->ptr, sizeof res);
    auto fresh = std::make_shared<ColStats>(ColStats{res.smin, res.smax, (int64_t)res.valid, res.valid > 0 && res.unsorted == 0, res.valid > 0 && res.descends == 0});
    std::atomic_store(&kc.stats, fresh);
    return *fresh;
  }
  return ColStats{res.smin, res.smax, 0, false, false};
}

static bool needs_visited(int join_type) {
  return join_type == DFGPU_JOIN_LEFT || join_type == DFGPU_JOIN_FULL || join_type == DFGPU_JOIN_LEFT_SEMI || join_type == DFGPU_JOIN_LEFT_ANTI ||
         join_type == DFGPU_JOIN_LEFT_MARK;
}

template <int KT>
__global__ void k_sample_near(KeyCol k, int64_t n, int64_t every, int samples, uint64_t window, int* __restrict__ near) {
  const int i = blockIdx.x * blockDim.x + threadIdx.x;
  if (i >= samples) return;
  const int64_t r = (int64_t)i * every;
  if (r + 1 >= n) return;
  const uint64_t a = load_key<KT>(k, r), b = load_key<KT>(k, r + 1);
  const uint64_t d = (int64_t)b >= (int64_t)a ? b - a : a - b;
  if (d <= window) atomicAdd(near, 1);
}
static bool probe_keys_clustered(const Column& kc, int64_t n, uint64_t window) {
  if (auto cached = std::atomic_load(&kc.stats))
    if (cached->nondecreasing) return true;
  if (n < (1 << 16) || !is_integer_like(kc.field.type) || kc.field.type == DFGPU_UINT64) return true;
  const uint64_t tag = (fmix64((uint64_t)kc.data_offset * 0x9E3779B97F4A7C15ull ^ (uint64_t)n ^ (window << 20)) & ~3ull) | 2ull;
  if (kc.data) {
    const uint64_t h = kc.data->hint.load(std::memory_order_relaxed);
    if ((h & ~1ull) == tag) return (h & 1ull) != 0;
  }
  constexpr int S = 4096;
  BufPtr cnt = make_zero_buf(4);
  const KeyCol k{kc.ptr(), nullptr, kc.field.type, type_width(kc.field.type)};
  with_key_type(k.type, [&](auto kt) { k_sample_near<decltype(kt)::value><<<S / BLOCK, BLOCK, 0, rt().stream>>>(k, n, n / S, S, window, cnt->as<int>()); });
  int near = 0;
  d2h(&near, cnt->ptr, 4);
  const bool clustered = near * 10 >= S * 9;
  if (kc.data) kc.data->hint.store(tag | (clustered ? 1ull : 0ull), std::memory_order_relaxed);
  return clustered;
}

static uint64_t all_hit_tag(const JoinTable& jt, const Table& probe, const std::vector<int>& pk, int kind) {
  uint64_t h = fmix64((uint64_t)probe.nrows * 0x9E3779B97F4A7C15ull ^ (uint64_t)jt.build.nrows ^ ((uint64_t)kind << 56));
  for (size_t i = 0; i < pk.size(); i++) {
    const Column& p = probe.cols[(size_t)pk[i]];
    const Column& b = jt.build.cols[(size_t)jt.key_cols[i]];
    h = fmix64(h ^ (uint64_t)(uintptr_t)p.ptr()) ^ fmix64((uint64_t)(uintptr_t)p.valid_words() + i);
    h = fmix64(h ^ (uint64_t)(uintptr_t)b.ptr()) ^ fmix64((uint64_t)(uintptr_t)b.valid_words() + 2 * i + 1);
  }
  return (h & ~3ull) | 2ull;
}

// ... 405 lines not shown
    }
  });
  DFGPU_HIP(hipGetLastError());
  launch.stop();
  unsigned missed = 0;
  if (box) {
    DFGPU_HIP(hipStreamSynchronize(r.stream));
    missed = *box->host;
  } else {
    d2h(&missed, miss_flag, 4);
  }
  if (missed) return probe_again_counted(p, spec, launch, out);
  for (int c : p.pout) {
    out.cols.push_back(p.probe.cols[c]);
    out.cols.back().length = np;
  }
  launch.record(p.plan.want_single ? "join_probe_fused" : "join_probe_placed", bytes);
  LateRecord::label("join_probe_shared_columns");
  out.nrows = np;
  return out;
}
static int64_t fused_counts_pass(ProbeRun& p, int64_t n_tiles, int invert, BufPtr& state, BufPtr& out_words) {
  Runtime& r = rt();
  ProbePlan& pl = p.plan;
  const int64_t np = p.np;
  BufPtr counts = make_buf((size_t)n_tiles * 4);
  state = make_buf((size_t)(n_tiles + 1) * 8);
  if (pl.listed) out_words = make_buf((size_t)p.n_words * 8);
  if (p.kind == KIND_RANK) {
    ensure_rank_bits(p.jt);
    p.ctx.rank_bits = p.jt.rank_bits->as<uint64_t>();
  }
  {
    ProfileScope ps("join_probe_tile_counts", pl.key_bytes + (pl.pred_in_counts ? np * p.lazy->pred_bytes_per_row : 0));
    with_kind_and_key(p.kind, p.ctx.pkeys.c[0].type, [&](auto kd, auto kt) {
      constexpr int K = decltype(kd)::value, T = decltype(kt)::value;
      uint64_t* const words = out_words ? out_words->as<uint64_t>() : nullptr;
      if constexpr (kind_is_direct<K>()) {
        const bool nt = option_on("join.counts_nt", true);
        if (pl.pred_in_counts) {
          if (nt) k_join_tile_counts<K, T, FUSED_W, true, true><<<(unsigned)n_tiles, BLOCK, 0, r.stream>>>(p.ctx, np, invert, nullptr, counts->as<uint32_t>(), words, p.lazy->pred);
          else k_join_tile_counts<K, T, FUSED_W, true><<<(unsigned)n_tiles, BLOCK, 0, r.stream>>>(p.ctx, np, invert, nullptr, counts->as<uint32_t>(), words, p.lazy->pred);
          return;
        }
        if (nt) {
          k_join_tile_counts<K, T, FUSED_W, false, true><<<(unsigned)n_tiles, BLOCK, 0, r.stream>>>(p.ctx, np, invert, p.row_mask, counts->as<uint32_t>(), words);
          return;
        }
      }
      k_join_tile_counts<K, T, FUSED_W><<<(unsigned)n_tiles, BLOCK, 0, r.stream>>>(p.ctx, np, invert, p.row_mask, counts->as<uint32_t>(), words);
    });
    DFGPU_HIP(hipGetLastError());
  }
  scan_u32(counts->as<uint32_t>(), n_tiles, state->as<uint64_t>());
  const int64_t n_alloc = (int64_t)read_u64(state->as<uint64_t>() + n_tiles);
  plan_after_counts(pl, n_alloc, np);
  if (!pl.listed) p.need_tab();
  if (pl.pred_in_counts && !pl.listed) p.set_row_mask(out_words->as<uint64_t>());
  return n_alloc;
}
static Table probe_fused(ProbeRun& p) {
  Runtime& r = rt();
  ProbePlan& pl = p.plan;
  const int64_t np = p.np, n_words = p.n_words;
  const int fused_mode = pl.fused_mode;
  const int64_t tile_words = (int64_t)FUSED_W * (BLOCK / WAVE), n_tiles = (n_words + tile_words - 1) / tile_words;
  const int invert = p.join_type == DFGPU_JOIN_RIGHT_ANTI;
  BufPtr state = fused_mode == FUSED_LOOKBACK ? make_zero_buf((size_t)n_tiles * 8) : nullptr;
  const Speculation spec = ask_all_hit(p, invert);
  if (spec.shared) return probe_shared(p, spec);
  BufPtr ctl = make_zero_buf(sizeof(FusedCtl));
  BufPtr out_words;
  const int64_t n_alloc = fused_mode == FUSED_PLACED && !spec.placed ? fused_counts_pass(p, n_tiles, invert, state, out_words) : np;
  const bool listed = pl.listed;
  Table out;
  JoinCopyCols jc{};
  jc.key_col = -1;
  const int64_t build_row_bytes = add_copy_cols(p.jt.build, p.bout, n_alloc, out, jc);
  jc.n_build = jc.n;
  if (pl.returned)
    for (int i = 0; i < jc.n_build; i++) {
      jc.src[i] = p.rp.rec->ptr;
      jc.ret_mul[i] = p.rp.mul[(size_t)i];
      jc.ret_add[i] = p.rp.add[(size_t)i];
    }
  const int64_t bytes_per_out = build_row_bytes + add_copy_cols(p.probe, p.pout, n_alloc, out, jc), bytes_build_once = p.jt.build.nrows * build_row_bytes;
  int64_t bytes_in = pl.key_bytes;
  for (size_t i = 0; i < p.pout.size(); i++) {
    const int c = p.pout[i], at = jc.n_build + (int)i;
    bool is_key = false;
    for (int k : p.pk) is_key |= k == c;
    if (!is_key) bytes_in += np * jc.width[at];
    if (is_key && (p.kind == KIND_ARRAY || p.kind == KIND_RANK) && p.pk.size() == 1 && jc.key_col < 0 && !p.probe.cols[c].validity) jc.key_col = at;
  }
  LateRecord launch;
  int64_t n_out = n_alloc;
  if (fused_mode != FUSED_PLACED || n_alloc > 0) {
    const unsigned g = fused_mode == FUSED_LOOKBACK ? (unsigned)std::min<int64_t>(n_tiles, (int64_t)r.num_cus * 8) : (unsigned)n_tiles;
    uint64_t* st = state ? state->as<uint64_t>() : nullptr;
    FusedCtl* const d_ctl = ctl->as<FusedCtl>();
    auto launch_fused = [&](auto kern) { kern<<<g, BLOCK, 0, r.stream>>>(p.ctx, jc, np, invert, st, d_ctl, p.row_mask); };
    with_kind_and_key(p.kind, p.ctx.pkeys.c[0].type, [&](auto kd, auto kt) {
      constexpr int K = decltype(kd)::value, T = decltype(kt)::value;
      constexpr bool KR = kind_is_direct<K>();
      if constexpr (KR) {
        if (listed) {
          const int64_t den = option_int("join.listed_sparse_den", 32);
          if (den > 0 && n_alloc * den <= np) {
// ... 1 lines not shown
            k_join_emit_listed<K, T, EL_WORDS_SPARSE><<<(unsigned)groups, BLOCK, 0, r.stream>>>(p.ctx, jc, np, out_words->as<uint64_t>(), st, (int)(EL_WORDS_SPARSE / tile_words));
          } else {
            const int64_t groups = (n_words + EL_WORDS - 1) / EL_WORDS;
            k_join_emit_listed<K, T, EL_WORDS><<<(unsigned)groups, BLOCK, 0, r.stream>>>(p.ctx, jc, np, out_words->as<uint64_t>(), st, (int)(EL_WORDS / tile_words));
          }
          return;
        }
      }
      if (fused_mode == FUSED_LOOKBACK) launch_fused(k_join_probe_fused<K, T, FUSED_W, FUSED_LOOKBACK, false>);
      else if (fused_mode == FUSED_PLACED && KR && jc.key_col >= 0) launch_fused(k_join_probe_fused<K, T, FUSED_W, FUSED_PLACED, KR>);
      else if (fused_mode == FUSED_PLACED) launch_fused(k_join_probe_fused<K, T, FUSED_W, FUSED_PLACED, false>);
      else if (KR && jc.key_col >= 0) launch_fused(k_join_probe_fused<K, T, FUSED_W, FUSED_UNORDERED, KR>);
      else launch_fused(k_join_probe_fused<K, T, FUSED_W, FUSED_UNORDERED, false>);
    });
    DFGPU_HIP(hipGetLastError());
    launch.stop();
    if (fused_mode != FUSED_PLACED) n_out = (int64_t)read_u64(reinterpret_cast<const uint64_t*>(&d_ctl->total));
    if (spec.placed) {
      unsigned missed = 0;
      d2h(&missed, &d_ctl->ticket, 4);
      if (missed) return probe_again_counted(p, spec, launch, out);
    }
  } else {
    launch.stop();
  }
  launch.record(listed ? "join_probe_listed" : fused_mode == FUSED_PLACED ? "join_probe_placed" : "join_probe_fused",
                bytes_in + (n_out > 0 ? bytes_build_once : 0) + n_out * bytes_per_out);
  out.nrows = n_out;
  for (Column& c : out.cols) c.length = n_out;
  return out;
}
static Table probe_first_match(ProbeRun& p) {
  Runtime& r = rt();
  const ProbePlan& pl = p.plan;
  const int64_t np = p.np, n_words = p.n_words;
  Table out;
  BufPtr mask = make_buf(bitmap_bytes(np));
  BufPtr first = pl.fast_inner ? make_buf((size_t)np * 4) : nullptr;
  {
    ProfileScope ps("join_probe_lookup", pl.key_bytes);
    const int g = grid_for(n_words, (BLOCK / WAVE) * PROBE_UNROLL), invert = p.join_type == DFGPU_JOIN_RIGHT_ANTI;
    with_kind_and_key(p.jt.kind, p.ctx.pkeys.c[0].type, [&](auto kd, auto kt) {
      k_probe_first<decltype(kd)::value, decltype(kt)::value><<<g, BLOCK, 0, r.stream>>>(p.ctx, np, invert, first ? first->as<uint32_t>() : nullptr,
                                                                                         mask->as<uint64_t>(), p.visited);
    });
    DFGPU_HIP(hipGetLastError());
  }
  if (pl.probe_side_only) return compact_table(p.probe, p.pout, mask->as<uint64_t>(), nullptr);
  if (pl.build_side_only) {
    for (int c : p.bout) out.cols.push_back(alloc_like(p.jt.build.cols[c], 0));
    return out;
  }
  BufPtr prefix = make_buf((size_t)(n_words + 1) * 8);
  scan_mask_popcounts(mask->as<uint64_t>(), nullptr, np, prefix->as<uint64_t>());
  const int64_t n_out = (int64_t)read_u64(prefix->as<uint64_t>() + n_words);
  out.nrows = n_out;
  JoinCopyCols jc{};
  int64_t bytes = 2 * n_out * add_copy_cols(p.jt.build, p.bout, n_out, out, jc);
  jc.n_build = jc.n;
  bytes += (np + n_out) * add_copy_cols(p.probe, p.pout, n_out, out, jc);
  if (n_out > 0 && jc.n > 0) {
    ProfileScope ps("join_probe_materialize", bytes);
    k_join_materialize<<<grid_for(n_words, (BLOCK / WAVE) * PROBE_UNROLL), BLOCK, 0, r.stream>>>(jc, mask->as<uint64_t>(), prefix->as<uint64_t>(),
                                                                                                  first->as<uint32_t>(), np);
    DFGPU_HIP(hipGetLastError());
  }
  return out;
}
static Table probe_pairs_single(ProbeRun& p) {
  Runtime& r = rt();
  const JoinTable& jt = p.jt;
  const int64_t np = p.np, n_words = p.n_words;
  constexpr int64_t SAMPLE = 1 << 16;
  const int64_t every = std::max<int64_t>(1, np / SAMPLE), n_sample = (np + every - 1) / every;
  BufPtr ctl = make_zero_buf(16);
  with_kind(jt.kind, [&](auto kt) {
    constexpr int K = decltype(kt)::value;
    if constexpr (kind_is_flat<K>()) k_probe_pairs_sample<K><<<grid_for(n_sample, BLOCK), BLOCK, 0, r.stream>>>(p.ctx, np, every, n_sample, ctl->as<unsigned long long>());
  });
  unsigned long long seen = 0;
  d2h(&seen, ctl->ptr, 8);
  unsigned long long capacity = (unsigned long long)((double)seen * (double)np / (double)n_sample * 1.25) + (1ull << 16);
  BufPtr ob, op;
  unsigned long long total = 0;
  for (int attempt = 0; attempt < 2; attempt++) {
    ob = make_buf((size_t)capacity * 8);
    op = make_buf((size_t)capacity * 8);
    DFGPU_HIP(hipMemsetAsync(ctl->ptr, 0, 16, r.stream));
    {
      ProfileScope ps("join_probe_pairs_single", p.plan.key_bytes + (int64_t)capacity * 16);
      const int g = (int)std::min<int64_t>((n_words + PROBE_UNROLL * (BLOCK / WAVE) - 1) / (PROBE_UNROLL * (BLOCK / WAVE)), (int64_t)r.num_cus * 16);
      with_kind(jt.kind, [&](auto kt) {
        constexpr int K = decltype(kt)::value;
        if constexpr (kind_is_flat<K>()) k_probe_pairs_single<K><<<g, BLOCK, 0, r.stream>>>(p.ctx, np, ctl->as<unsigned long long>(), capacity, ob->as<int64_t>(), op->as<int64_t>());
      });
      DFGPU_HIP(hipGetLastError());
    }
    d2h(&total, ctl->ptr, 8);
    if (total <= capacity) break;
    DFGPU_CHECK(attempt == 0, "join: the single-pass probe overflowed a buffer of its exact size");
    capacity = total;
  }
  Table out;
  out.nrows = (int64_t)total;
  for (Column& c : gather_columns(jt.build, p.bout, ob->as<int64_t>(), out.nrows, false)) out.cols.push_back(std::move(c));
  for (Column& c : gather_columns(p.probe, p.pout, op->as<int64_t>(), out.nrows, false)) out.cols.push_back(std::move(c));
  return out;
}
static Table probe_pairs(ProbeRun& p) {
  Runtime& r = rt();
  const int join_type = p.join_type;
  const int64_t np = p.np, n_words = p.n_words, key_bytes = p.plan.key_bytes;
  BufPtr row_counts = make_buf((size_t)(np ? np : 1) * 4);
  BufPtr row_first = make_buf((size_t)(np ? np : 1) * 4);
  BufPtr word_counts = make_buf((size_t)(n_words ? n_words : 1) * 4);
  BufPtr prefix = make_buf((size_t)(n_words + 1) * 8);
  int g = grid_for(n_words, BLOCK / WAVE);
  if (np) {
    ProfileScope ps("join_probe_count", key_bytes + np * 4);
    with_kind(p.jt.kind, [&](auto kt) {
      k_probe_count<decltype(kt)::value><<<g, BLOCK, 0, r.stream>>>(p.ctx, np, join_type, row_counts->as<uint32_t>(), word_counts->as<uint32_t>(), p.visited, row_first->as<uint32_t>());
    });
    DFGPU_HIP(hipGetLastError());
  }
  scan_u32(word_counts->as<uint32_t>(), n_words, prefix->as<uint64_t>());
  const int64_t n_out = (int64_t)read_u64(prefix->as<uint64_t>() + n_words);
  BufPtr ob = make_buf((size_t)(n_out ? n_out : 1) * 8), op = make_buf((size_t)(n_out ? n_out : 1) * 8);
  BufPtr om = join_type == DFGPU_JOIN_RIGHT_MARK ? make_buf((size_t)n_out + 64) : nullptr;
  if (n_out) {
    ProfileScope ps("join_probe_emit", key_bytes + np * 4 + n_out * 16);
    with_kind(p.jt.kind, [&](auto kt) {
      k_probe_emit<decltype(kt)::value><<<g, BLOCK, 0, r.stream>>>(p.ctx, np, join_type, row_counts->as<uint32_t>(), prefix->as<uint64_t>(), ob->as<int64_t>(), op->as<int64_t>(), om ? om->as<uint8_t>() : nullptr, row_first->as<uint32_t>());
    });
    DFGPU_HIP(hipGetLastError());
  }
  Table out;
  out.nrows = n_out;
  const bool build_null_possible = join_type == DFGPU_JOIN_RIGHT || join_type == DFGPU_JOIN_FULL;
  if (join_type != DFGPU_JOIN_RIGHT_MARK)
    for (Column& c : gather_columns(p.jt.build, p.bout, ob->as<int64_t>(), n_out, build_null_possible)) out.cols.push_back(std::move(c));
  for (Column& c : gather_columns(p.probe, p.pout, op->as<int64_t>(), n_out, false)) out.cols.push_back(std::move(c));
  if (join_type == DFGPU_JOIN_RIGHT_MARK) out.cols.push_back(mark_column(om->as<uint8_t>(), n_out));
  return out;
}
static Table probe_core(JoinTable& jt, const Table& probe, const std::vector<int>& pk, int join_type, const std::vector<int>& bout, const std::vector<int>& pout,
                        const uint64_t* row_mask, bool* mask_consumed, const LazyRowFilter* lazy, ProbeHints hints, uint8_t* visited) {
  ProbeRun p{jt, probe, pk, join_type, bout, pout, row_mask, lazy, mask_consumed, hints, visited, probe.nrows, (probe.nrows + 63) / 64, jt.kind,
             make_ctx(jt, probe, pk, false, false),
             {}, {}};
  p.ctx.row_mask = row_mask;
  ProbePlan& pl = p.plan = plan_probe(p);
  if (trace_on("join"))
    fprintf(stderr, "[dfgpu join_probe] np=%lld kind=%d probe_mode=%d fused_ok=%d big_table=%d unclustered=%d grouped_keys_only=%d returned=%d rows_unused=%d row_mask=%d\n",
            (long long)p.np, jt.kind, jt.probe_mode, pl.fused_ok, pl.big_table, pl.unclustered, pl.grouped_keys_only, pl.try_returned, pl.rows_unused, row_mask != nullptr);
  if (pl.try_returned) {
    p.need_mask();
    plan_after_lookup(pl, p, grouped_probe_lookup(jt, probe, pk[0], bout, p.row_mask, p.rp));
  }
  if (pl.returned) {
    p.kind = KIND_RETURNED;
    p.ctx.ret_dest = p.rp.dest->as<uint32_t>();
    p.ctx.ret_rec = p.rp.rec->as<uint8_t>();
    p.ctx.ret_R = p.rp.R;
  } else if (!pl.rows_unused && jt.kind == KIND_RANK && jt.rank_needs_perm) {
    ensure_rank_perm(jt);
    p.ctx.rank_perm = jt.rank_perm->as<uint32_t>();
    p.ctx.rank_tab = jt.rank_tab->as<ulonglong2>();
  }
  DFGPU_CHECK(!((jt.probe_mode == 2 || jt.probe_mode == 3) && !pl.fused_ok),
              "single-pass probe requested but not applicable (needs <=1 match per probe row and non-nullable payload)");
  if (pl.grouped_keys_only) return probe_grouped_keys(p);
  pl.pred_in_counts = p.lazy != nullptr && pl.use_fused && pl.listed;
  if (!pl.pred_in_counts) p.need_mask();
  if (p.row_mask || pl.pred_in_counts) {
    DFGPU_CHECK(mask_consumed != nullptr, "probe row mask without a fallback");
    *mask_consumed = pl.use_fused || pl.one_match_path;
    if (!*mask_consumed) return Table{};
  }
  if (!(pl.use_fused && pl.listed && p.kind == KIND_RANK)) p.need_tab();
// ... 51 lines not shown

static Table empty_selection(const Table& t, const std::vector<int>& cols) {
  BufPtr zero = make_zero_buf(bitmap_bytes(t.nrows));
  return compact_table(t, cols, zero->as<uint64_t>(), nullptr);
}

static Table join_probe_null_aware(JoinTable& jt, const Table& probe, const std::vector<int>& pk, int join_type, const std::vector<int>& bout,
                                   const std::vector<int>& pout) {
  switch (null_aware_before_probe(jt, probe, pk, join_type, false)) {
    case NA_EMPTY:
      for (int c : pout) DFGPU_CHECK(c >= 0 && c < (int)probe.cols.size(), "probe output column out of range");
      {
        std::lock_guard<std::mutex> lk(jt.mu);
        jt.info.probe_rows += probe.nrows;
      }
      return empty_selection(probe, pout);
    case NA_MASK_NULL_PROBE_KEYS: {
      bool consumed = false;
      Table res = join_probe(jt, probe, pk, join_type, bout, pout, probe.cols[pk[0]].valid_words(), &consumed);
      if (!consumed) {
        std::vector<int> all(probe.cols.size());
        for (size_t i = 0; i < all.size(); i++) all[i] = (int)i;
        const Table filtered = compact_table(probe, all, probe.cols[pk[0]].valid_words(), nullptr);
        res = join_probe(jt, filtered, pk, join_type, bout, pout);
      }
      return res;
    }
    default:
      return join_probe(jt, probe, pk, join_type, bout, pout);
  }
}

struct Pairs {
  BufPtr ob, op;
  int64_t m = 0;
};
static Pairs key_equal_pairs(JoinTable& jt, const Table& probe, const std::vector<int>& pk) {
  Runtime& r = rt();
  Pairs P;
  if (jt.kind == KIND_RADIX) {
    radix_join_pairs(*jt.radix, jt.build, jt.key_cols, probe, pk, jt.null_equality == DFGPU_NULL_EQUALS_NULL, jt.force_collisions, P.ob, P.op, P.m);
    return P;
  }
  const int64_t np = probe.nrows;
  const int64_t n_words = (np + 63) / 64;
  ProbeCtx ctx = make_ctx(jt, probe, pk);
  BufPtr row_counts = make_buf((size_t)(np ? np : 1) * 4), word_counts = make_buf((size_t)(n_words ? n_words : 1) * 4);
  BufPtr row_first = make_buf((size_t)(np ? np : 1) * 4);
  BufPtr prefix = make_buf((size_t)(n_words + 1) * 8);
  const int g = grid_for(n_words, BLOCK / WAVE);
  if (np) with_kind(jt.kind, [&](auto kt) {
    k_probe_count<decltype(kt)::value><<<g, BLOCK, 0, r.stream>>>(ctx, np, DFGPU_JOIN_INNER, row_counts->as<uint32_t>(), word_counts->as<uint32_t>(), nullptr, row_first->as<uint32_t>());
  });
  scan_u32(word_counts->as<uint32_t>(), n_words, prefix->as<uint64_t>());
  P.m = (int64_t)read_u64(prefix->as<uint64_t>() + n_words);
  P.ob = make_buf((size_t)(P.m ? P.m : 1) * 8);
  P.op = make_buf((size_t)(P.m ? P.m : 1) * 8);
  if (P.m) with_kind(jt.kind, [&](auto kt) {
    k_probe_emit<decltype(kt)::value><<<g, BLOCK, 0, r.stream>>>(ctx, np, DFGPU_JOIN_INNER, row_counts->as<uint32_t>(), prefix->as<uint64_t>(), P.ob->as<int64_t>(), P.op->as<int64_t>(), nullptr, row_first->as<uint32_t>());
  });
  DFGPU_HIP(hipGetLastError());
  return P;
}

void join_bytes_mask(const uint8_t* bytes, int64_t n, bool want_set, uint64_t* mask) {
  if (n) k_visited_mask<<<grid_for((n + 63) / 64, BLOCK / WAVE), BLOCK, 0, rt().stream>>>(bytes, n, want_set ? 1 : 0, mask);
  DFGPU_HIP(hipGetLastError());
}
void join_append_unmatched(const uint64_t* mask, const uint64_t* prefix, int64_t n, int64_t base, int64_t* null_side, int64_t* row_side) {
  if (n) k_append_unmatched<<<grid_for((n + 63) / 64, BLOCK / WAVE), BLOCK, 0, rt().stream>>>(mask, prefix, n, base, null_side, row_side);
  DFGPU_HIP(hipGetLastError());
}
void join_pairs_compact(const int64_t* ob, const int64_t* op, const uint64_t* pass, const uint64_t* prefix, int64_t m, int64_t* ob2, int64_t* op2) {
  if (m) k_pairs_compact<<<grid_for((m + 63) / 64, BLOCK / WAVE), BLOCK, 0, rt().stream>>>(ob, op, pass, prefix, m, ob2, op2);
  DFGPU_HIP(hipGetLastError());
}

static Table join_probe_with_filter(JoinTable& jt, const Table& probe, const std::vector<int>& pk, int join_type, const std::vector<int>& bout,
                                    const std::vector<int>& pout, const dfgpu_join_filter* jfp) {
  Runtime& r = rt();
  DFGPU_CHECK(pk.size() == jt.key_cols.size(), "probe key count differs from build key count");
  DFGPU_CHECK(probe.device == jt.build.device, "the probe table lives on another device than the join table (move it with dfgpu_table_copy_to_device)");
  for (int c : bout) DFGPU_CHECK(c >= 0 && c < (int)jt.build.cols.size(), "build output column out of range");
  for (int c : pout) DFGPU_CHECK(c >= 0 && c < (int)probe.cols.size(), "probe output column out of range");
  const int64_t np = probe.nrows;
  const int64_t n_words = (np + 63) / 64;
  const int g = grid_for(n_words, BLOCK / WAVE);
  {
    std::lock_guard<std::mutex> lk(jt.mu);
    jt.info.probe_rows += np;
  }
  Pairs P = key_equal_pairs(jt, probe, pk);
  const int64_t m = P.m;
  BufPtr ob = P.ob, op = P.op;
  if (!jfp && join_type == DFGPU_JOIN_INNER) {
    Table out;
    out.nrows = m;
    for (Column& c : gather_columns(jt.build, bout, ob->as<int64_t>(), m, false)) out.cols.push_back(std::move(c));
    for (Column& c : gather_columns(probe, pout, op->as<int64_t>(), m, false)) out.cols.push_back(std::move(c));
    DFGPU_HIP(hipStreamSynchronize(r.stream));
    jt.info.output_rows += out.nrows;
    return out;
  }
  const int64_t m_words = (m + 63) / 64;
  BufPtr pass = make_buf((size_t)(m_words ? m_words : 1) * 8);
  DFGPU_HIP(hipMemsetAsync(pass->ptr, jfp ? 0 : 0xFF, (size_t)(m_words ? m_words : 1) * 8, r.stream));
  if (m && jfp) {
    const dfgpu_join_filter& jf = *jfp;
    Table inter;
    inter.nrows = m;
    for (int i = 0; i < jf.n_columns; i++) {
      const bool left = jf.column_side[i] == 0;
      const Table& side = left ? jt.build : probe;
      DFGPU_CHECK(jf.column_index[i] >= 0 && jf.column_index[i] < (int)side.cols.size(), "join filter column index out of range");
      inter.cols.push_back(gather_column(side.cols[jf.column_index[i]], (left ? ob : op)->as<int64_t>(), m, false));
    }
    Datum d = evaluate(jf.expression, inter);
    DFGPU_CHECK(d.col.field.type == DFGPU_BOOL, "join filter expression must be Boolean");
    Column mc = datum_to_column(d, m, "");
    if (mc.validity) and_bitmaps(mc.data->as<uint64_t>(), mc.valid_words(), m_words, pass->as<uint64_t>());
    else pass = mc.data;
  }
  BufPtr hits = make_zero_buf((size_t)(np ? np : 1) * 4);
  uint8_t* visited = nullptr;
  if (needs_visited(join_type)) {
    {
      std::lock_guard<std::mutex> lk(jt.mu);
      if (!jt.visited) {
        jt.visited = make_zero_buf((size_t)jt.build.nrows + 64);
        DFGPU_HIP(hipStreamSynchronize(rt().stream));
      }
    }
    visited = jt.visited->as<uint8_t>();
  }
  if (m) k_pair_tally<<<grid_for(m, BLOCK), BLOCK, 0, r.stream>>>(ob->as<int64_t>(), op->as<int64_t>(), pass->as<uint64_t>(), m, hits->as<uint32_t>(), visited);
  Table out;
  const bool pairs_out = join_type == DFGPU_JOIN_INNER || join_type == DFGPU_JOIN_LEFT || join_type == DFGPU_JOIN_RIGHT || join_type == DFGPU_JOIN_FULL;
  if (pairs_out) {
    BufPtr pprefix = make_buf((size_t)(m_words + 1) * 8);
    scan_mask_popcounts(pass->as<uint64_t>(), nullptr, m, pprefix->as<uint64_t>());
    const int64_t n_pass = m ? (int64_t)read_u64(pprefix->as<uint64_t>() + m_words) : 0;
    int64_t n_un = 0;
    BufPtr umask, uprefix;
    const bool probe_outer = join_type == DFGPU_JOIN_RIGHT || join_type == DFGPU_JOIN_FULL;
    if (probe_outer && np) {
      umask = make_buf(bitmap_bytes(np));
      uprefix = make_buf((size_t)(n_words + 1) * 8);
      k_hits_mask<<<g, BLOCK, 0, r.stream>>>(hits->as<uint32_t>(), np, 0, umask->as<uint64_t>(), nullptr);
      scan_mask_popcounts(umask->as<uint64_t>(), nullptr, np, uprefix->as<uint64_t>());
      n_un = (int64_t)read_u64(uprefix->as<uint64_t>() + n_words);
    }
    const int64_t n_out = n_pass + n_un;
    BufPtr ob2 = make_buf((size_t)(n_out ? n_out : 1) * 8), op2 = make_buf((size_t)(n_out ? n_out : 1) * 8);
    if (n_pass) k_pairs_compact<<<grid_for(m_words, BLOCK / WAVE), BLOCK, 0, r.stream>>>(ob->as<int64_t>(), op->as<int64_t>(), pass->as<uint64_t>(), pprefix->as<uint64_t>(), m,
                                                                                        ob2->as<int64_t>(), op2->as<int64_t>());
    if (n_un) k_append_unmatched<<<g, BLOCK, 0, r.stream>>>(umask->as<uint64_t>(), uprefix->as<uint64_t>(), np, n_pass, ob2->as<int64_t>(), op2->as<int64_t>());
    DFGPU_HIP(hipGetLastError());
    out.nrows = n_out;
    for (Column& c : gather_columns(jt.build, bout, ob2->as<int64_t>(), n_out, probe_outer)) out.cols.push_back(std::move(c));
    for (Column& c : gather_columns(probe, pout, op2->as<int64_t>(), n_out, false)) out.cols.push_back(std::move(c));
  } else if (join_type == DFGPU_JOIN_RIGHT_SEMI || join_type == DFGPU_JOIN_RIGHT_ANTI) {
    BufPtr mask = make_zero_buf(bitmap_bytes(np ? np : 1));
    if (np) k_hits_mask<<<g, BLOCK, 0, r.stream>>>(hits->as<uint32_t>(), np, join_type == DFGPU_JOIN_RIGHT_SEMI, mask->as<uint64_t>(), nullptr);
    out = compact_table(probe, pout, mask->as<uint64_t>(), nullptr);
  } else if (join_type == DFGPU_JOIN_RIGHT_MARK) {
    BufPtr mask = make_zero_buf(bitmap_bytes(np ? np : 1));
    BufPtr bytes = make_zero_buf((size_t)np + 64);
    if (np) k_hits_mask<<<g, BLOCK, 0, r.stream>>>(hits->as<uint32_t>(), np, 1, mask->as<uint64_t>(), bytes->as<uint8_t>());
    out.nrows = np;
    for (int c : pout) out.cols.push_back(probe.cols[c]);
    out.cols.push_back(mark_column(bytes->as<uint8_t>(), np));
  } else {
    out.nrows = 0;
    for (int c : bout) out.cols.push_back(alloc_like(jt.build.cols[c], 0));
  }
  DFGPU_HIP(hipStreamSynchronize(r.stream));
  jt.info.output_rows += out.nrows;
  return out;
}

}

using namespace dfgpu;

extern "C" {

int dfgpu_join_build(dfgpu_table_t build, const int* key_cols, int nkeys, int null_equality, const dfgpu_join_options* opts, dfgpu_join_t* out) {
  return guarded([&] {
    require_init();
    DFGPU_CHECK(nkeys >= 1 && key_cols && out, "join needs at least one key column");
    dfgpu_join_options o{1024, DFGPU_DEFAULT_MIN_KEY_DENSITY, 0, 0, 0, 0};
    if (opts) o = *opts;
    auto jt = join_build(*unwrap(build), std::vector<int>(key_cols, key_cols + nkeys), null_equality, o);
    *out = reinterpret_cast<dfgpu_join_t>(jt.release());
  });
}

struct JoinBuilder {
  std::vector<int> key_cols;
  int null_equality = 0;
  dfgpu_join_options opts{};
  std::vector<std::unique_ptr<Table>> batches;
  int64_t rows = 0, bytes = 0;
// ... 489 lines not shown
```

datafusion_amd/csrc/runtime.hip:

```cpp
#include "internal.hpp"

#include <chrono>
#include <algorithm>
#include <cstring>
#include <atomic>

namespace dfgpu {

static thread_local std::string g_last_error;
void set_last_error(const std::string& msg) { g_last_error = msg; }

static std::mutex g_devices_mu;
static std::vector<std::unique_ptr<Runtime>> g_runtimes;
static std::vector<int> g_initialised;
static Runtime g_uninitialised;
static thread_local int t_device = -1;
static thread_local int t_hip_device = -1;

const std::vector<int>& initialised_devices() { return g_initialised; }
int current_device() {
  if (t_device >= 0) return t_device;
  return g_initialised.empty() ? -1 : g_initialised[0];
}
Runtime& rt_of(int device) {
  DFGPU_CHECK(device >= 0 && device < (int)g_runtimes.size() && g_runtimes[device] && g_runtimes[device]->initialised,
              "device " + std::to_string(device) + " has not been initialised (dfgpu_init)");
  return *g_runtimes[device];
}
void use_device(int device) {
  if (device == t_device && device == t_hip_device) return;
  (void)rt_of(device);
  if (t_hip_device != device) {
    DFGPU_HIP(hipSetDevice(device));
    t_hip_device = device;
  }
  t_device = device;
}
Runtime& rt() {
  const int d = current_device();
  if (d < 0) return g_uninitialised;
  if (t_hip_device != d) {
    if (hipSetDevice(d) == hipSuccess) t_hip_device = d;
    else (void)hipGetLastError();
  }
  return *g_runtimes[d];
}
void require_init() { DFGPU_CHECK(rt().initialised, "dfgpu_init() has not been called"); }
static std::mutex g_opt_mu;
static std::map<std::string, std::string> g_options;
const Policy& policy() { return rt().policy; }
static bool env_option(const char* name, std::string& out) {
  const char* e = std::getenv("DFGPU_OPTIONS");
// ... 226 lines not shown

DevBuf::DevBuf(size_t n) : bytes(n), owner(&rt()) { ptr = owner->alloc(n); }
DevBuf::~DevBuf() {
  if (owner) owner->free(ptr);
}

BufPtr make_zero_buf(size_t bytes) {
  BufPtr b = make_buf(bytes);
  DFGPU_HIP(hipMemsetAsync(b->ptr, 0, bytes ? bytes : 1, rt().stream));
  return b;
}

void d2h(void* dst, const void* src, size_t n) {
  constexpr size_t PIN = 64 << 10;
  static thread_local void* t_pin = nullptr;
  if (n <= PIN && option_on("runtime.pinned_readback", true)) {
    if (!t_pin && hipHostMalloc(&t_pin, PIN, hipHostMallocDefault) != hipSuccess) {
      (void)hipGetLastError();
      t_pin = nullptr;
    }
    if (t_pin) {
      DFGPU_HIP(hipMemcpyAsync(t_pin, src, n, hipMemcpyDeviceToHost, rt().stream));
      DFGPU_HIP(hipStreamSynchronize(rt().stream));
      std::memcpy(dst, t_pin, n);
      return;
    }
  }
  DFGPU_HIP(hipMemcpyAsync(dst, src, n, hipMemcpyDeviceToHost, rt().stream));
  DFGPU_HIP(hipStreamSynchronize(rt().stream));
}
HostFlag* thread_host_flag() {
  if (!option_on("runtime.pinned_readback", true)) return nullptr;
  struct Slot { HostFlag f; bool failed = false; };
  static thread_local std::vector<Slot> t_flags;
  const int d = rt().device;
  if (d < 0) return nullptr;
  if ((int)t_flags.size() <= d) t_flags.resize((size_t)d + 1);
  Slot& s = t_flags[(size_t)d];
  if (s.failed) return nullptr;
  if (!s.f.host) {
    void* h = nullptr;
    void* dev = nullptr;
    if (hipHostMalloc(&h, 64, hipHostMallocDefault) != hipSuccess || hipHostGetDevicePointer(&dev, h, 0) != hipSuccess || !dev) {
      (void)hipGetLastError();
      if (h) (void)hipHostFree(h);
      s.failed = true;
      return nullptr;
    }
    s.f.host = static_cast<volatile unsigned*>(h);
    s.f.dev = static_cast<unsigned*>(dev);
    *s.f.host = 0u;
  }
  return &s.f;
}
void h2d_async(void* dst, const void* src, size_t n) {
  DFGPU_HIP(hipMemcpyAsync(dst, src, n, hipMemcpyHostToDevice, rt().stream));
}
uint64_t read_u64(const uint64_t* dev) {
  uint64_t v = 0;
  d2h(&v, dev, 8);
  return v;
}

dfgpu_metrics& thread_metrics() {
  static thread_local dfgpu_metrics m{};
  return m;
}

ProfileScope::ProfileScope(const char* n, int64_t algorithmic_bytes) : name(n), bytes(algorithmic_bytes) {
  Runtime& r = rt();
  thread_metrics().hbm_bytes_algorithmic += algorithmic_bytes;
  if (!r.profiling) return;
  (void)hipEventCreate(&a);
  (void)hipEventCreate(&b);
  (void)hipEventRecord(a, r.stream);
}
ProfileScope::~ProfileScope() {
  if (!a) return;
  Runtime& r = rt();
  (void)hipEventRecord(b, r.stream);
  std::lock_guard<std::mutex> lk(r.mu);
  r.recs.push_back({name, a, b, bytes, std::this_thread::get_id()});
}
LateRecord::LateRecord() {
  Runtime& r = rt();
  if (!r.profiling) return;
  DFGPU_HIP(hipEventCreate(&a));
  DFGPU_HIP(hipEventCreate(&b));
  DFGPU_HIP(hipEventRecord(a, r.stream));
}
LateRecord::~LateRecord() {
  if (a) (void)hipEventDestroy(a);
  if (b) (void)hipEventDestroy(b);
}
void LateRecord::stop() {
  if (a) DFGPU_HIP(hipEventRecord(b, rt().stream));
}
void LateRecord::record(const char* name, int64_t algorithmic_bytes) {
  if (!a) return;
  Runtime& r = rt();
  std::lock_guard<std::mutex> lk(r.mu);
  r.recs.push_back({name, a, b, algorithmic_bytes, std::this_thread::get_id()});
  a = b = nullptr;
}
void LateRecord::label(const char* name) {
  Runtime& r = rt();
// ... 365 lines not shown
```

datafusion_amd/csrc/scan.hip:

```cpp
#include "device.hpp"
#include "internal.hpp"

namespace dfgpu {

constexpr int SCAN_ITEMS = 8;
constexpr int SCAN_CHUNK = BLOCK * SCAN_ITEMS;

struct InU32 {
  const uint32_t* p;
  __device__ __forceinline__ uint32_t operator()(int64_t i) const { return p[i]; }
};
struct InMaskPopc {
  const uint64_t* mask;
  const uint64_t* valid;
  int64_t nrows;
  __device__ __forceinline__ uint32_t operator()(int64_t w) const {
    uint64_t m = mask[w];
    if (valid) m &= valid[w];
    int64_t rem = nrows - w * 64;
    if (rem < 64) m &= (rem <= 0) ? 0ull : ((~0ull) >> (64 - rem));
    return (uint32_t)__popcll(m);
  }
};

__device__ __forceinline__ uint64_t block_exclusive_scan(uint64_t v, uint64_t* total) {
  __shared__ uint64_t wsum[BLOCK / WAVE];
  uint64_t inc = wave_inclusive_sum(v);
  int w = threadIdx.x >> 6;
  if (lane_id() == 63) wsum[w] = inc;
  __syncthreads();
  uint64_t base = 0, tot = 0;
#pragma unroll
  for (int i = 0; i < BLOCK / WAVE; i++) {
    if (i < w) base += wsum[i];
    tot += wsum[i];
  }
  __syncthreads();
  *total = tot;
  return base + inc - v;
}

template <typename In>
__global__ __launch_bounds__(BLOCK) void k_scan_reduce(In in, int64_t n, uint64_t* chunk_sums) {
  int64_t base = (int64_t)blockIdx.x * SCAN_CHUNK + (int64_t)threadIdx.x * SCAN_ITEMS;
  uint64_t s = 0;
#pragma unroll
  for (int j = 0; j < SCAN_ITEMS; j++)
    if (base + j < n) s += in(base + j);
  uint64_t tot;
  block_exclusive_scan(s, &tot);
  if (threadIdx.x == 0) chunk_sums[blockIdx.x] = tot;
}

__global__ __launch_bounds__(BLOCK) void k_scan_sums(uint64_t* sums, int64_t n_chunks, uint64_t* total) {
  uint64_t carry = 0;
  for (int64_t base = 0; base < n_chunks; base += BLOCK) {
    int64_t i = base + threadIdx.x;
    uint64_t v = i < n_chunks ? sums[i] : 0;
    uint64_t tot;
    uint64_t ex = block_exclusive_scan(v, &tot);
    if (i < n_chunks) sums[i] = carry + ex;
    carry += tot;
  }
  if (threadIdx.x == 0) *total = carry;
}

template <typename In>
__global__ __launch_bounds__(BLOCK) void k_scan_down(In in, int64_t n, const uint64_t* chunk_base, uint64_t* out) {
  int64_t base = (int64_t)blockIdx.x * SCAN_CHUNK + (int64_t)threadIdx.x * SCAN_ITEMS;
  uint32_t v[SCAN_ITEMS];
  uint64_t s = 0;
#pragma unroll
  for (int j = 0; j < SCAN_ITEMS; j++) {
    v[j] = base + j < n ? in(base + j) : 0;
    s += v[j];
  }
  uint64_t tot;
  uint64_t ex = block_exclusive_scan(s, &tot) + chunk_base[blockIdx.x];
#pragma unroll
  for (int j = 0; j < SCAN_ITEMS; j++) {
    if (base + j < n) out[base + j] = ex;
    ex += v[j];
  }
}

constexpr int CH_ITEMS = 16;
constexpr int CH_CHUNK = BLOCK * CH_ITEMS;
template <typename In>
__global__ __launch_bounds__(BLOCK) void k_scan_chained(In in, int64_t n, uint64_t* __restrict__ state, unsigned* __restrict__ ticket, uint64_t* __restrict__ out) {
  __shared__ unsigned s_tile;
  __shared__ uint64_t s_excl;
  if (threadIdx.x == 0) s_tile = atomicAdd(ticket, 1u);
  __syncthreads();
  const int64_t tile = s_tile;
  const int64_t n_tiles = (n + CH_CHUNK - 1) / CH_CHUNK;
  const int64_t base = tile * CH_CHUNK + (int64_t)threadIdx.x * CH_ITEMS;
  uint32_t v[CH_ITEMS];
  uint64_t s = 0;
#pragma unroll
  for (int j = 0; j < CH_ITEMS; j++) {
    v[j] = base + j < n ? in(base + j) : 0;
    s += v[j];
  }
  uint64_t tot;
  uint64_t ex = block_exclusive_scan(s, &tot);
  if (threadIdx.x < WAVE) {
    const uint64_t excl = lookback_exclusive(state, tile, tot);
    if (threadIdx.x == 0) {
      s_excl = excl;
      if (tile == n_tiles - 1) out[n] = excl + tot;
    }
  }
  __syncthreads();
  ex += s_excl;
#pragma unroll
  for (int j = 0; j < CH_ITEMS; j++) {
    if (base + j < n) out[base + j] = ex;
    ex += v[j];
  }
}

template <typename In>
static void run_scan(In in, int64_t n, uint64_t* out, const char* name) {
  Runtime& r = rt();
  if (n == 0) {
    DFGPU_HIP(hipMemsetAsync(out, 0, 8, r.stream));
    return;
  }
  const int64_t n_tiles_ch = (n + CH_CHUNK - 1) / CH_CHUNK;
  if (n_tiles_ch <= option_int("scan.chained_max_tiles", 8)) {
    const int64_t n_tiles = n_tiles_ch;
    BufPtr state = make_zero_buf((size_t)(n_tiles + 2) * 8);
    ProfileScope ps(name, 0);
    k_scan_chained<<<(unsigned)n_tiles, BLOCK, 0, r.stream>>>(in, n, state->as<uint64_t>(), reinterpret_cast<unsigned*>(state->as<uint64_t>() + n_tiles), out);
    DFGPU_HIP(hipGetLastError());
    return;
  }
  int64_t n_chunks = (n + SCAN_CHUNK - 1) / SCAN_CHUNK;
  BufPtr sums = make_buf((size_t)n_chunks * 8);
  ProfileScope ps(name, 0);
  k_scan_reduce<<<(unsigned)n_chunks, BLOCK, 0, r.stream>>>(in, n, sums->as<uint64_t>());
  k_scan_sums<<<1, BLOCK, 0, r.stream>>>(sums->as<uint64_t>(), n_chunks, out + n);
  k_scan_down<<<(unsigned)n_chunks, BLOCK, 0, r.stream>>>(in, n, sums->as<uint64_t>(), out);
  DFGPU_HIP(hipGetLastError());
}

void scan_mask_popcounts(const uint64_t* mask, const uint64_t* valid, int64_t nrows, uint64_t* out_prefix) {
  int64_t n_words = (nrows + 63) / 64;
  run_scan(InMaskPopc{mask, valid, nrows}, n_words, out_prefix, "scan_mask_popcounts");
}
void scan_u32(const uint32_t* in, int64_t n, uint64_t* out_prefix) { run_scan(InU32{in}, n, out_prefix, "scan_u32"); }

}
```

datafusion_amd/csrc/sort.hip:

```cpp
#include <algorithm>
#include <cstdlib>

#include "device.hpp"
#include "internal.hpp"
#include "onesweep.hpp"
#include "records.hpp"

namespace dfgpu {

constexpr int MAX_SORT_KEYS = 8;
constexpr int MAX_KEY_WORDS = 3;

struct PackCol {
  const void* data;
  const uint64_t* valid;
  int type;
  int desc;
  int nulls_first;
  int has_null_bit;
  uint64_t base_lo, base_hi;
  int bits;
  int shift;
  uint64_t mult, range;
};
// ... 1872 lines not shown
  BufPtr a0, a1, b0, b1;
  if (dg.n > 1) {
    a0 = make_buf((size_t)n * 16 + 64);
    if (w2) a1 = make_buf((size_t)n * w2 + 64);
  }
  if (dg.n > 2) {
    b0 = make_buf((size_t)n * 16 + 64);
    if (w2) b1 = make_buf((size_t)n * w2 + 64);
  }
  const int grid = (int)std::min<int64_t>(n_tiles, (int64_t)r.num_cus * 4);
  LsdIo io{};
  for (int p = 0; p < dg.n; p++) {
    const bool first = p == 0, last = p == dg.n - 1;
    if (!last) {
      const bool to_a = first || io.in0 == b0->as<uint4>();
      io.out0 = (to_a ? a0 : b0)->as<uint4>();
      io.out1 = w2 ? (to_a ? a1 : b1)->ptr : nullptr;
    }
    ProfileScope ps(last ? "sort_lsd_pass_out" : "sort_lsd_pass", n * (int64_t)((first ? row_bytes : rec_bytes) + (last ? row_bytes : rec_bytes)));
    if (!ahead) DFGPU_HIP(hipMemsetAsync(state->ptr, 0, (size_t)n_tiles * 256 * 4, r.stream));
    auto launch = [&](auto kern) {
      kern<<<grid, BLOCK, 0, r.stream>>>(io, kc, L, key_off, n, reverse, dg.shift[p], dg.bits[p], n_tiles, ahead ? nullptr : bases->as<unsigned long long>() + p * 256,
                                         ahead ? nullptr : state->as<uint32_t>(), tickets->as<unsigned>() + p, e, ah[ahead ? p : 0]);
    };
    auto pick = [&](auto w2c) {
      constexpr int W2 = decltype(w2c)::value;
      if (ahead) {
        if (first) launch(k_lsd_pass<true, false, W2, true>);
        else launch(k_lsd_pass<false, true, W2, true>);
      } else if (first && last) launch(k_lsd_pass<true, true, W2>);
      else if (first) launch(k_lsd_pass<true, false, W2>);
      else if (last) launch(k_lsd_pass<false, true, W2>);
      else launch(k_lsd_pass<false, false, W2>);
    };
    if (w2 == 0) pick(std::integral_constant<int, 0>{});
    else if (w2 == 8) pick(std::integral_constant<int, 8>{});
    else pick(std::integral_constant<int, 16>{});
    DFGPU_HIP(hipGetLastError());
    io.in0 = io.out0;
    io.in1 = io.out1;
  }
  DFGPU_HIP(hipStreamSynchronize(r.stream));
  return true;
}

struct Survivors {
  SortedKeys keys;
  BufPtr remap;
  int64_t m = 0;
};
static BufPtr compact_mask(const BufPtr& mask, int64_t n, int64_t at_least, int64_t at_most, int64_t& m) {
  const int64_t n_words = (n + 63) / 64;
  BufPtr prefix = make_buf((size_t)(n_words + 1) * 8);
  scan_mask_popcounts(mask->as<uint64_t>(), nullptr, n, prefix->as<uint64_t>());
  m = (int64_t)read_u64(prefix->as<uint64_t>() + n_words);
  if (m < at_least || m > at_most) return nullptr;
  BufPtr ids = make_buf((size_t)(m ? m : 1) * 8);
  mask_to_ids(mask->as<uint64_t>(), prefix->as<uint64_t>(), n, m, ids->as<int64_t>());
  return ids;
}

static Survivors topk_by_sampled_limit(const KeyPlan& kp, int64_t n, int64_t n_out) {
  Runtime& r = rt();
  const PackCols& pc = kp.pc;
  const int64_t S = 1 << 14, every = n / S;
  const int64_t c = std::min<int64_t>(S, (n_out * S + n - 1) / n * 2 + 16);
  if (!kp.narrow || n < (1 << 20) || c >= S / 4) return {};
  BufPtr d_sample = make_buf((size_t)S * 8);
  const int64_t n_words = (n + 63) / 64;
  BufPtr mask = make_buf(bitmap_bytes(n));
  const int top_shift = kp.total_bits > 0 ? ((std::min(kp.total_bits, 64) - 1) / 8) * 8 : 0;
  BufPtr d_limit = make_buf(16);
  uint64_t* limit = d_limit->as<uint64_t>();
  {
    ProfileScope ps("topk_limit_sample", S * 16);
    k_pack_keys64_rows<<<grid_for(S, BLOCK), BLOCK, 0, r.stream>>>(pc, nullptr, every, S, d_sample->as<uint64_t>());
    k_select_kth<<<1, SELECT_THREADS, 0, r.stream>>>(d_sample->as<uint64_t>(), S, c, top_shift, limit);
    DFGPU_HIP(hipGetLastError());
  }
  {
    ProfileScope ps("topk_limit_pass", kp.key_col_bytes + n / 8);
    bool plain_keys = n < ((int64_t)1 << 32);
    for (int k = 0; k < pc.n; k++) plain_keys = plain_keys && key_reads_back(pc.c[k]);
    if (plain_keys) k_key_limit_mask_plain<<<grid_for(n_words, (BLOCK / WAVE) * 4), BLOCK, 0, r.stream>>>(pc, n, limit, mask->as<uint64_t>());
    else k_key_limit_mask<<<grid_for(n_words, BLOCK / WAVE), BLOCK, 0, r.stream>>>(pc, n, limit, mask->as<uint64_t>());
    DFGPU_HIP(hipGetLastError());
  }
  Survivors sv;
  sv.remap = compact_mask(mask, n, n_out, std::max<int64_t>(1 << 22, 64 * n_out), sv.m);
  if (!sv.remap) return {};
  sv.keys = one_word_keys(make_buf((size_t)sv.m * 8));
  k_pack_keys64_rows<<<grid_for(sv.m, BLOCK), BLOCK, 0, r.stream>>>(pc, sv.remap->as<int64_t>(), 0, sv.m, sv.keys.w[0]->as<uint64_t>());
  sv.keys.idx = iota_ids(sv.m);
  DFGPU_HIP(hipGetLastError());
  if (sv.m > SMALL_SORT_CAP && sv.m <= ((int64_t)1 << 22) && option_on("sort.topk_second_narrowing", true)) {
    BufPtr cursor = make_zero_buf(4);
    const SortedKeys s2 = one_word_keys(make_buf((size_t)SMALL_SORT_CAP * 8), make_buf((size_t)SMALL_SORT_CAP * 4));
    {
      ProfileScope ps("topk_second_narrowing", sv.m * 8 * 2);
      const int64_t S2 = std::min<int64_t>(S, sv.m), every2 = sv.m / S2;
      const int64_t c2 = std::min<int64_t>(S2, (n_out * S2 + sv.m - 1) / sv.m * 2 + 16);
      k_strided_u64<<<grid_for(S2, BLOCK), BLOCK, 0, r.stream>>>(sv.keys.w[0]->as<uint64_t>(), every2, S2, d_sample->as<uint64_t>());
      k_select_kth<<<1, SELECT_THREADS, 0, r.stream>>>(d_sample->as<uint64_t>(), S2, c2, top_shift, limit + 1);
      k_take_le<<<grid_for(sv.m, BLOCK * 4), BLOCK, 0, r.stream>>>(sv.keys.w[0]->as<uint64_t>(), sv.m, limit + 1, cursor->as<unsigned>(), SMALL_SORT_CAP, s2.w[0]->as<uint64_t>(),
                                                                    s2.idx->as<uint32_t>());
      DFGPU_HIP(hipGetLastError());
    }
    unsigned taken = 0;
// ... 145 lines not shown
```

Baseline: 346.1 billion rows/s.

## Return small kernel results through mapped host slots instead of blocking d2h copies

Adds a ring of pinned, mapped, coherent host memory slots that kernels write their scalar answers into with a system-scope release store. The host spin-waits on a sequence word instead of issuing a synchronous device-to-host copy. This is applied to scan totals, key min/max, the key-ends speculation check and the speculation verify flag. The key-ends kernel also becomes a single 1024-thread block with a shared-memory reduction. The aim is to cut the per-readback latency of full stream syncs and small memcpys on the join build path. In exchange it adds host CPU spinning, fallback complexity and reliance on coherent mapped memory.

```diff
diff --git a/datafusion_amd/csrc/aggregate.hip b/datafusion_amd/csrc/aggregate.hip
--- a/datafusion_amd/csrc/aggregate.hip
+++ b/datafusion_amd/csrc/aggregate.hip
@@ -1717,8 +1717,9 @@
   BufPtr prefix = make_buf((size_t)(n_words + 1) * 8);
   const uint64_t n_slots = cap + (keyed ? 1 : 0);
   k_mark_reps<<<grid_for((int64_t)n_slots, BLOCK), BLOCK, 0, r.stream>>>(R.slots->as<uint32_t>(), n_slots, rep_mask->as<unsigned long long>());
-  scan_mask_popcounts(rep_mask->as<uint64_t>(), nullptr, total, prefix->as<uint64_t>());
-  R.G1 = (int64_t)read_u64(prefix->as<uint64_t>() + n_words);
+  ScanTotal scan_total;
+  scan_mask_popcounts(rep_mask->as<uint64_t>(), nullptr, total, prefix->as<uint64_t>(), &scan_total);
+  R.G1 = (int64_t)scan_total.get();
   R.slot_gid = make_buf((cap + 1) * 4);
   BufPtr rep_row = make_buf((size_t)(R.G1 ? R.G1 : 1) * 8);
   k_slot_gids<<<grid_for((int64_t)n_slots, BLOCK), BLOCK, 0, r.stream>>>(R.slots->as<uint32_t>(), n_slots, rep_mask->as<uint64_t>(), prefix->as<uint64_t>(),
@@ -3276,8 +3277,9 @@
   if (by_parts && pv.rep_mask) {
     const int64_t row_words = (n + 63) / 64;
     BufPtr rprefix = make_buf((size_t)(row_words + 1) * 8);
-    scan_mask_popcounts(pv.rep_mask->as<uint64_t>(), nullptr, n, rprefix->as<uint64_t>());
-    const int64_t G = (int64_t)read_u64(rprefix->as<uint64_t>() + row_words);
+    ScanTotal scan_total;
+    scan_mask_popcounts(pv.rep_mask->as<uint64_t>(), nullptr, n, rprefix->as<uint64_t>(), &scan_total);
+    const int64_t G = (int64_t)scan_total.get();
     grow_accumulators(A, 0, G, false);
     const DenseEmit e = dense_emit_of();
     int kci = -1;
@@ -3316,8 +3318,9 @@
     ProfileScope ps("agg_dense_setbits", key_bytes);
     jit_launch(f_setbits, grid, BLOCK, 0, &args, sizeof(args));
   }
-  scan_mask_popcounts(bits->as<uint64_t>(), nullptr, n_words * 64, prefix->as<uint64_t>());
-  const int64_t Gk = (int64_t)read_u64(prefix->as<uint64_t>() + n_words);
+  ScanTotal scan_total;
+  scan_mask_popcounts(bits->as<uint64_t>(), nullptr, n_words * 64, prefix->as<uint64_t>(), &scan_total);
+  const int64_t Gk = (int64_t)scan_total.get();
   const int64_t G = Gk + (null_group ? 1 : 0);
   BufPtr first_row = make_buf((size_t)std::max<int64_t>(G, 1) * 4);
   BufPtr seen = by_parts ? make_buf((size_t)std::max<int64_t>(G, 1) * 4) : make_zero_buf((size_t)std::max<int64_t>(G, 1) * 4);
@@ -3349,8 +3352,9 @@
   BufPtr rep_mask = make_zero_buf((size_t)row_words * 8);
   BufPtr rprefix = make_buf((size_t)(row_words + 1) * 8);
   if (G) k_mark_first_rows<<<grid_for(G, BLOCK), BLOCK, 0, r.stream>>>(first_row->as<uint32_t>(), G, rep_mask->as<unsigned long long>());
-  scan_mask_popcounts(rep_mask->as<uint64_t>(), nullptr, n, rprefix->as<uint64_t>());
-  DFGPU_CHECK((int64_t)read_u64(rprefix->as<uint64_t>() + row_words) == G, "dense-key node: first-row marks do not match the group count");
+  ScanTotal marks_total;
+  scan_mask_popcounts(rep_mask->as<uint64_t>(), nullptr, n, rprefix->as<uint64_t>(), &marks_total);
+  DFGPU_CHECK((int64_t)marks_total.get() == G, "dense-key node: first-row marks do not match the group count");
   grow_accumulators(A, 0, G, false);
   const DenseEmit e = dense_emit_of();
   BufPtr new_gid = make_buf((size_t)std::max<int64_t>(G, 1) * 4);
@@ -3705,8 +3709,6 @@
     }
     DFGPU_HIP(hipGetLastError());
   }
-  BufPtr prefix = make_buf((size_t)(n_words + 1) * 8);
-  scan_mask_popcounts(heads->as<uint64_t>(), nullptr, n, prefix->as<uint64_t>());
   BufPtr long_flag = make_zero_buf(8);
   k_run_long_flag<<<grid_for(n_words, BLOCK), BLOCK, 0, r.stream>>>(heads->as<uint64_t>(), n_words, long_flag->as<uint32_t>());
   if (!more_keys.empty()) {
@@ -3726,9 +3728,12 @@
     }
     DFGPU_HIP(hipGetLastError());
   }
-  const int64_t G = (int64_t)read_u64(prefix->as<uint64_t>() + n_words);
+  BufPtr prefix = make_buf((size_t)(n_words + 1) * 8);
+  ScanTotal scan_total;
+  scan_mask_popcounts(heads->as<uint64_t>(), nullptr, n, prefix->as<uint64_t>(), &scan_total, long_flag->as<uint64_t>());
+  const int64_t G = (int64_t)scan_total.get();
   uint32_t flags[2] = {0, 0};
-  d2h(flags, long_flag->ptr, 8);
+  std::memcpy(flags, &scan_total.carried, 8);
   if (flags[1]) return false;
   const uint32_t has_long = flags[0];
   fix_argument_types(A, cp, arg_out);
diff --git a/datafusion_amd/csrc/device.hpp b/datafusion_amd/csrc/device.hpp
--- a/datafusion_amd/csrc/device.hpp
+++ b/datafusion_amd/csrc/device.hpp
@@ -232,6 +232,14 @@
   if (b > 256 * 8) b = 256 * 8;
   return (int)b;
 }
+
+constexpr int HOST_SLOT_WORDS = 8, HOST_SLOT_PAYLOAD = 6, HOST_SLOT_SEQ = 7;
+__device__ __forceinline__ void host_slot_post(uint64_t* slot, uint64_t seq, const uint64_t* payload, int n_words) {
+  if (!slot) return;
+  for (int i = 0; i < n_words && i < HOST_SLOT_PAYLOAD; i++) slot[i] = payload[i];
+  __hip_atomic_store(slot + HOST_SLOT_SEQ, seq, __ATOMIC_RELEASE, __HIP_MEMORY_SCOPE_SYSTEM);
+}
+__device__ __forceinline__ void host_slot_post(uint64_t* slot, uint64_t seq, uint64_t value) { host_slot_post(slot, seq, &value, 1); }
 
 constexpr uint64_t TS_AGG = 1ull << 62, TS_PFX = 2ull << 62, TS_VAL = (1ull << 62) - 1;
 
diff --git a/datafusion_amd/csrc/filter.hip b/datafusion_amd/csrc/filter.hip
--- a/datafusion_amd/csrc/filter.hip
+++ b/datafusion_amd/csrc/filter.hip
@@ -149,8 +149,9 @@
   const int64_t n_words = (n + 63) / 64;
   Table out;
   BufPtr prefix = make_buf((size_t)(n_words + 1) * 8);
-  scan_mask_popcounts(mask, mask_valid, n, prefix->as<uint64_t>());
-  const int64_t n_out = (int64_t)read_u64(prefix->as<uint64_t>() + n_words);
+  ScanTotal total;
+  scan_mask_popcounts(mask, mask_valid, n, prefix->as<uint64_t>(), &total);
+  const int64_t n_out = (int64_t)total.get();
   out.nrows = n_out;
   std::vector<BufPtr> valid_bytes(cols.size());
   for (size_t i = 0; i < cols.size(); i++) {
diff --git a/datafusion_amd/csrc/internal.hpp b/datafusion_amd/csrc/internal.hpp
--- a/datafusion_amd/csrc/internal.hpp
+++ b/datafusion_amd/csrc/internal.hpp
@@ -173,6 +173,19 @@
   unsigned* dev = nullptr;
 };
 HostFlag* thread_host_flag();
+constexpr int HOST_SLOT_RING = 64;
+constexpr int64_t HOST_SLOT_SPIN_US = 1000;
+constexpr int64_t HOST_SLOT_QUERY_US = 5;
+struct HostSlot {
+  uint64_t* dev = nullptr;
+  const volatile uint64_t* host = nullptr;
+  uint64_t seq = 0;
+  explicit operator bool() const { return dev != nullptr; }
+};
+HostSlot host_slot_acquire();
+void host_slot_wait(const HostSlot& s, void* dst, size_t n);
+inline int host_slot_index(uint64_t use) { return (int)(use % HOST_SLOT_RING); }
+inline uint64_t host_slot_seq(uint64_t use) { return use; }
 extern std::atomic<int64_t> g_pinned_driver_allocs, g_pinned_driver_ns;
 void* pinned_alloc(size_t n);
 void pinned_release(void* p);
@@ -291,8 +304,16 @@
 
 inline dfgpu_table_t wrap_quiet(Table* t) { return reinterpret_cast<dfgpu_table_t>(t); }
 
-void scan_mask_popcounts(const uint64_t* mask, const uint64_t* valid, int64_t nrows, uint64_t* out_prefix);
-void scan_u32(const uint32_t* in, int64_t n, uint64_t* out_prefix);
+struct ScanTotal {
+  HostSlot slot;
+  const uint64_t* dev_word = nullptr;
+  const uint64_t* carry = nullptr;
+  uint64_t value = 0, carried = 0;
+  bool known = false;
+  uint64_t get();
+};
+void scan_mask_popcounts(const uint64_t* mask, const uint64_t* valid, int64_t nrows, uint64_t* out_prefix, ScanTotal* total = nullptr, const uint64_t* carry = nullptr);
+void scan_u32(const uint32_t* in, int64_t n, uint64_t* out_prefix, ScanTotal* total = nullptr);
 uint64_t read_u64(const uint64_t* dev);
 
 Table compact_table(const Table& in, const std::vector<int>& cols, const uint64_t* mask, const uint64_t* mask_valid);
diff --git a/datafusion_amd/csrc/join.hip b/datafusion_amd/csrc/join.hip
--- a/datafusion_amd/csrc/join.hip
+++ b/datafusion_amd/csrc/join.hip
@@ -162,7 +162,7 @@
 };
 constexpr int BUILD_UNROLL = 4;
 template <int KT, bool HASV>
-__global__ __launch_bounds__(BLOCK) void k_key_minmax(KeyCol k, int64_t n, MinMax* out) {
+__global__ __launch_bounds__(BLOCK) void k_key_minmax(KeyCol k, int64_t n, MinMax* out, unsigned* done, uint64_t* slot, uint64_t slot_seq) {
   long long mn = INT64_MAX, mx = INT64_MIN;
   unsigned long long cnt = 0;
   bool unsorted = false, descends = false;
@@ -229,20 +229,38 @@
     }
     if (uns & 1u) atomicOr(&out->unsorted, 1u);
     if (uns & 2u) atomicOr(&out->descends, 1u);
+    if (slot && __hip_atomic_fetch_add(done, 1u, __ATOMIC_RELEASE, __HIP_MEMORY_SCOPE_AGENT) == gridDim.x - 1) {
+      __builtin_amdgcn_fence(__ATOMIC_ACQUIRE, "agent");
+      const uint64_t answer[4] = {(uint64_t)__hip_atomic_load(&out->smin, __ATOMIC_RELAXED, __HIP_MEMORY_SCOPE_AGENT),
+                                  (uint64_t)__hip_atomic_load(&out->smax, __ATOMIC_RELAXED, __HIP_MEMORY_SCOPE_AGENT),
+                                  __hip_atomic_load(&out->valid, __ATOMIC_RELAXED, __HIP_MEMORY_SCOPE_AGENT),
+                                  (uint64_t)__hip_atomic_load(&out->unsorted, __ATOMIC_RELAXED, __HIP_MEMORY_SCOPE_AGENT) |
+                                      (uint64_t)__hip_atomic_load(&out->descends, __ATOMIC_RELAXED, __HIP_MEMORY_SCOPE_AGENT) << 32};
+      host_slot_post(slot, slot_seq, answer, 4);
+    }
   }
 }
 
 template <int KT>
-__global__ void k_key_ends(KeyCol k, int64_t n, int64_t every, int samples, long long* __restrict__ out) {
-  const int i = blockIdx.x * blockDim.x + threadIdx.x;
-  if (i == 0) {
-    out[0] = (long long)load_key<KT>(k, 0);
-    out[1] = (long long)load_key<KT>(k, n - 1);
-  }
-  if (i >= samples) return;
-  const int64_t r = (int64_t)i * every;
-  if (r + 1 >= n) return;
-  if ((long long)load_key<KT>(k, r + 1) <= (long long)load_key<KT>(k, r)) atomicOr((unsigned long long*)&out[2], 1ull);
+__global__ __launch_bounds__(1024) void k_key_ends(KeyCol k, int64_t n, int64_t every, int samples, long long* __restrict__ out, uint64_t* slot, uint64_t slot_seq) {
+  __shared__ int s_bad;
+  if (threadIdx.x == 0) s_bad = 0;
+  __syncthreads();
+  bool bad = false;
+#pragma unroll 4
+  for (int i = threadIdx.x; i < samples; i += blockDim.x) {
+    const int64_t r = (int64_t)i * every;
+    if (r + 1 < n) bad |= (long long)load_key<KT>(k, r + 1) <= (long long)load_key<KT>(k, r);
+  }
+  if (ballot64(bad) != 0 && lane_id() == 0) s_bad = 1;
+  __syncthreads();
+  if (threadIdx.x == 0) {
+    const long long e[3] = {(long long)load_key<KT>(k, 0), (long long)load_key<KT>(k, n - 1), (long long)s_bad};
+    out[0] = e[0];
+    out[1] = e[1];
+    out[2] = e[2];
+    host_slot_post(slot, slot_seq, reinterpret_cast<const uint64_t*>(e), 3);
+  }
 }
 
 template <int KT, bool HASV, bool ASCENDING, bool VERIFY = false>
@@ -1809,6 +1827,33 @@
     default: throw Error("key type has no direct-address instantiation");
   }
 }
+struct MinMaxBlock {
+  MinMax m{INT64_MAX, INT64_MIN, 0, 0, 0};
+  unsigned done = 0, pad = 0;
+};
+static_assert(sizeof(MinMax) == 32, "k_key_minmax posts a MinMax as four words");
+static MinMax run_key_minmax(const KeyCol& k, int64_t n, const char* record) {
+  Runtime& r = rt();
+  BufPtr mm = make_buf(sizeof(MinMaxBlock));
+  static const MinMaxBlock init;
+  h2d_async(mm->ptr, &init, sizeof init);
+  const HostSlot slot = host_slot_acquire();
+  {
+    ProfileScope ps(record, n * k.width);
+    const int g = std::min(grid_for(n, BLOCK * BUILD_UNROLL), 512);
+    MinMaxBlock* const d = mm->as<MinMaxBlock>();
+    with_key_type(k.type, [&](auto kt) {
+      constexpr int T = decltype(kt)::value;
+      if (k.valid) k_key_minmax<T, true><<<g, BLOCK, 0, r.stream>>>(k, n, &d->m, &d->done, slot.dev, slot.seq);
+      else k_key_minmax<T, false><<<g, BLOCK, 0, r.stream>>>(k, n, &d->m, &d->done, slot.dev, slot.seq);
+    });
+    DFGPU_HIP(hipGetLastError());
+  }
+  MinMax res;
+  if (slot) host_slot_wait(slot, &res, sizeof res);
+  else d2h(&res, mm->ptr, sizeof res);
+  return res;
+}
 template <typename F>
 static void with_kind_and_key(int kind, int probe_key_type, F&& f) {
   if (kind == KIND_HASH) {
@@ -2038,10 +2083,13 @@
   if (!known && speculate && !spec_off && (opts.table_mode == 0 || opts.table_mode == 3) && ks.n == 1 && is_integer_like(ks.c[0].type) && ks.c[0].type != DFGPU_UINT64 &&
       !ks.c[0].valid && nb >= (1 << 22)) {
     constexpr int S = 4096;
-    BufPtr ends = make_zero_buf(24);
-    with_key_type(ks.c[0].type, [&](auto kt) { k_key_ends<decltype(kt)::value><<<S / BLOCK, BLOCK, 0, r.stream>>>(ks.c[0], nb, nb / S, S, ends->as<long long>()); });
+    BufPtr ends = make_buf(24);
+    const HostSlot slot = host_slot_acquire();
+    with_key_type(ks.c[0].type, [&](auto kt) { k_key_ends<decltype(kt)::value><<<1, 1024, 0, r.stream>>>(ks.c[0], nb, nb / S, S, ends->as<long long>(), slot.dev, slot.seq); });
+    DFGPU_HIP(hipGetLastError());
     long long e[3] = {0, 0, 1};
-    d2h(e, ends->ptr, 24);
+    if (slot) host_slot_wait(slot, e, 24);
+    else d2h(e, ends->ptr, 24);
     const uint64_t grange = (uint64_t)e[1] - (uint64_t)e[0];
     if (e[2] == 0 && e[1] > e[0] && grange != UINT64_MAX && grange + 1 >= (uint64_t)nb && grange < (1ull << 40)) {
       const double gdense = (double)nb / ((double)grange + 1.0);
@@ -2059,20 +2107,7 @@
     const Column& kc = build.cols[key_cols[0]];
     bool null_block = null_equality == DFGPU_NULL_EQUALS_NULL && kc.has_nulls();
     if (!null_block && nb > 0) {
-      BufPtr mm = make_buf(sizeof(MinMax));
-      static const MinMax init{INT64_MAX, INT64_MIN, 0, 0, 0};
-      h2d_async(mm->ptr, &init, sizeof init);
-      {
-        ProfileScope ps("join_build_key_stats", nb * ks.c[0].width);
-        const int g = std::min(grid_for(nb, BLOCK * BUILD_UNROLL), 512);
-        with_key_type(ks.c[0].type, [&](auto kt) {
-          constexpr int T = decltype(kt)::value;
-          if (ks.c[0].valid) k_key_minmax<T, true><<<g, BLOCK, 0, r.stream>>>(ks.c[0], nb, mm->as<MinMax>());
-          else k_key_minmax<T, false><<<g, BLOCK, 0, r.stream>>>(ks.c[0], nb, mm->as<MinMax>());
-        });
-      }
-      MinMax res;
-      d2h(&res, mm->ptr, sizeof res);
+      const MinMax res = run_key_minmax(ks.c[0], nb, "join_build_key_stats");
       n_valid_keys = (int64_t)res.valid;
       if (res.valid > 0) {
         range = (uint64_t)res.smax - (uint64_t)res.smin;
@@ -2096,7 +2131,7 @@
 
   BufPtr flag;
   auto need_flag = [&]() {
-    if (!flag) flag = make_zero_buf(4);
+    if (!flag) flag = make_zero_buf(8);
     return flag->as<int>();
   };
   int dup = 0;
@@ -2123,6 +2158,8 @@
   if (rank_ok) {
     const int64_t n_words = (int64_t)(range >> 6) + 1;
     BufPtr eager_tab;
+    int verify_word = 0;
+    bool verify_known = false;
     if (ascending && (double)nb >= 0.15 * ((double)range + 1.0)) {
       const bool no_fill = known && known->ascending && known->valid == nb && known->onepass_fit == (RT_FIT_TAG | 1ull) && option_on("join.onepass_no_fill", true);
       eager_tab = no_fill ? make_buf((size_t)n_words * 16) : make_zero_buf((size_t)n_words * 16);
@@ -2202,12 +2239,20 @@
       }
     }
     jt->rank_prefix = make_buf((size_t)(n_words + 1) * 8);
-    scan_mask_popcounts(jt->rank_bits->as<uint64_t>(), nullptr, n_words * 64, jt->rank_prefix->as<uint64_t>());
-    if (!ascending) dup = (int64_t)read_u64(jt->rank_prefix->as<uint64_t>() + n_words) != n_valid_keys;
+    ScanTotal bits_total;
+    const bool ask = !ascending || speculated;
+    scan_mask_popcounts(jt->rank_bits->as<uint64_t>(), nullptr, n_words * 64, jt->rank_prefix->as<uint64_t>(), ask ? &bits_total : nullptr,
+                        speculated ? reinterpret_cast<const uint64_t*>(need_flag()) : nullptr);
+    if (!ascending) dup = (int64_t)bits_total.get() != n_valid_keys;
+    if (speculated && bits_total.slot) {
+      bits_total.get();
+      verify_word = (int)(uint32_t)bits_total.carried;
+      verify_known = true;
+    }
     }
     if (speculated) {
-      int wrong = 0;
-      d2h(&wrong, need_flag(), 4);
+      int wrong = verify_word;
+      if (!verify_known) d2h(&wrong, need_flag(), 4);
       if (wrong & 1) {
         ProfileScope ps("join_build_speculation_missed", 0);
         jt.reset();
@@ -2393,23 +2438,10 @@
 ColStats column_stats(Column& kc, int64_t nrows) {
   DFGPU_CHECK(is_integer_like(kc.field.type) && kc.field.type != DFGPU_UINT64, "dfgpu_column_minmax: integer columns only");
   if (auto cached = std::atomic_load(&kc.stats)) return *cached;
-  Runtime& r = rt();
   MinMax res{INT64_MAX, INT64_MIN, 0, 0, 0};
   if (nrows > 0) {
     KeyCol k{kc.ptr(), kc.valid_words(), kc.field.type, type_width(kc.field.type)};
-    BufPtr mm = make_buf(sizeof(MinMax));
-    h2d_async(mm->ptr, &res, sizeof res);
-    {
-      ProfileScope ps("column_minmax", nrows * k.width);
-      const int g = std::min(grid_for(nrows, BLOCK * BUILD_UNROLL), 512);
-      with_key_type(k.type, [&](auto kt) {
-        constexpr int T = decltype(kt)::value;
-        if (k.valid) k_key_minmax<T, true><<<g, BLOCK, 0, r.stream>>>(k, nrows, mm->as<MinMax>());
-        else k_key_minmax<T, false><<<g, BLOCK, 0, r.stream>>>(k, nrows, mm->as<MinMax>());
-      });
-      DFGPU_HIP(hipGetLastError());
-    }
-    d2h(&res, mm->ptr, sizeof res);
+    res = run_key_minmax(k, nrows, "column_minmax");
     auto fresh = std::make_shared<ColStats>(ColStats{res.smin, res.smax, (int64_t)res.valid, res.valid > 0 && res.unsorted == 0, res.valid > 0 && res.descends == 0});
     std::atomic_store(&kc.stats, fresh);
     return *fresh;
@@ -2921,8 +2953,9 @@
     });
     DFGPU_HIP(hipGetLastError());
   }
-  scan_u32(counts->as<uint32_t>(), n_tiles, state->as<uint64_t>());
-  const int64_t n_alloc = (int64_t)read_u64(state->as<uint64_t>() + n_tiles);
+  ScanTotal scan_total;
+  scan_u32(counts->as<uint32_t>(), n_tiles, state->as<uint64_t>(), &scan_total);
+  const int64_t n_alloc = (int64_t)scan_total.get();
   plan_after_counts(pl, n_alloc, np);
   if (!pl.listed) p.need_tab();
   if (pl.pred_in_counts && !pl.listed) p.set_row_mask(out_words->as<uint64_t>());
@@ -3030,8 +3063,9 @@
     return out;
   }
   BufPtr prefix = make_buf((size_t)(n_words + 1) * 8);
-  scan_mask_popcounts(mask->as<uint64_t>(), nullptr, np, prefix->as<uint64_t>());
-  const int64_t n_out = (int64_t)read_u64(prefix->as<uint64_t>() + n_words);
+  ScanTotal scan_total;
+  scan_mask_popcounts(mask->as<uint64_t>(), nullptr, np, prefix->as<uint64_t>(), &scan_total);
+  const int64_t n_out = (int64_t)scan_total.get();
   out.nrows = n_out;
   JoinCopyCols jc{};
   int64_t bytes = 2 * n_out * add_copy_cols(p.jt.build, p.bout, n_out, out, jc);
@@ -3101,8 +3135,9 @@
     });
     DFGPU_HIP(hipGetLastError());
   }
-  scan_u32(word_counts->as<uint32_t>(), n_words, prefix->as<uint64_t>());
-  const int64_t n_out = (int64_t)read_u64(prefix->as<uint64_t>() + n_words);
+  ScanTotal scan_total;
+  scan_u32(word_counts->as<uint32_t>(), n_words, prefix->as<uint64_t>(), &scan_total);
+  const int64_t n_out = (int64_t)scan_total.get();
   BufPtr ob = make_buf((size_t)(n_out ? n_out : 1) * 8), op = make_buf((size_t)(n_out ? n_out : 1) * 8);
   BufPtr om = join_type == DFGPU_JOIN_RIGHT_MARK ? make_buf((size_t)n_out + 64) : nullptr;
   if (n_out) {
@@ -3260,8 +3295,9 @@
   if (np) with_kind(jt.kind, [&](auto kt) {
     k_probe_count<decltype(kt)::value><<<g, BLOCK, 0, r.stream>>>(ctx, np, DFGPU_JOIN_INNER, row_counts->as<uint32_t>(), word_counts->as<uint32_t>(), nullptr, row_first->as<uint32_t>());
   });
-  scan_u32(word_counts->as<uint32_t>(), n_words, prefix->as<uint64_t>());
-  P.m = (int64_t)read_u64(prefix->as<uint64_t>() + n_words);
+  ScanTotal scan_total;
+  scan_u32(word_counts->as<uint32_t>(), n_words, prefix->as<uint64_t>(), &scan_total);
+  P.m = (int64_t)scan_total.get();
   P.ob = make_buf((size_t)(P.m ? P.m : 1) * 8);
   P.op = make_buf((size_t)(P.m ? P.m : 1) * 8);
   if (P.m) with_kind(jt.kind, [&](auto kt) {
@@ -3346,8 +3382,9 @@
   const bool pairs_out = join_type == DFGPU_JOIN_INNER || join_type == DFGPU_JOIN_LEFT || join_type == DFGPU_JOIN_RIGHT || join_type == DFGPU_JOIN_FULL;
   if (pairs_out) {
     BufPtr pprefix = make_buf((size_t)(m_words + 1) * 8);
-    scan_mask_popcounts(pass->as<uint64_t>(), nullptr, m, pprefix->as<uint64_t>());
-    const int64_t n_pass = m ? (int64_t)read_u64(pprefix->as<uint64_t>() + m_words) : 0;
+    ScanTotal scan_total;
+    scan_mask_popcounts(pass->as<uint64_t>(), nullptr, m, pprefix->as<uint64_t>(), &scan_total);
+    const int64_t n_pass = m ? (int64_t)scan_total.get() : 0;
     int64_t n_un = 0;
     BufPtr umask, uprefix;
     const bool probe_outer = join_type == DFGPU_JOIN_RIGHT || join_type == DFGPU_JOIN_FULL;
@@ -3355,8 +3392,9 @@
       umask = make_buf(bitmap_bytes(np));
       uprefix = make_buf((size_t)(n_words + 1) * 8);
       k_hits_mask<<<g, BLOCK, 0, r.stream>>>(hits->as<uint32_t>(), np, 0, umask->as<uint64_t>(), nullptr);
-      scan_mask_popcounts(umask->as<uint64_t>(), nullptr, np, uprefix->as<uint64_t>());
-      n_un = (int64_t)read_u64(uprefix->as<uint64_t>() + n_words);
+      ScanTotal scan_total;
+      scan_mask_popcounts(umask->as<uint64_t>(), nullptr, np, uprefix->as<uint64_t>(), &scan_total);
+      n_un = (int64_t)scan_total.get();
     }
     const int64_t n_out = n_pass + n_un;
     BufPtr ob2 = make_buf((size_t)(n_out ? n_out : 1) * 8), op2 = make_buf((size_t)(n_out ? n_out : 1) * 8);
diff --git a/datafusion_amd/csrc/runtime.hip b/datafusion_amd/csrc/runtime.hip
--- a/datafusion_amd/csrc/runtime.hip
+++ b/datafusion_amd/csrc/runtime.hip
@@ -1,3 +1,4 @@
+#include "device.hpp"
 #include "internal.hpp"
 
 #include <chrono>
@@ -330,6 +331,81 @@
     *s.f.host = 0u;
   }
   return &s.f;
+}
+namespace {
+struct SlotRing {
+  uint64_t* host = nullptr;
+  uint64_t* dev = nullptr;
+  uint64_t uses = 0;
+  bool failed = false;
+};
+inline void cpu_pause() {
+#if defined(__x86_64__) || defined(__i386__)
+  __builtin_ia32_pause();
+#else
+  std::this_thread::yield();
+#endif
+}
+}
+HostSlot host_slot_acquire() {
+  if (!option_on("runtime.pinned_readback", true)) return {};
+  static thread_local std::vector<SlotRing> t_rings;
+  const int d = rt().device;
+  if (d < 0) return {};
+  if ((int)t_rings.size() <= d) t_rings.resize((size_t)d + 1);
+  SlotRing& g = t_rings[(size_t)d];
+  if (g.failed) return {};
+  if (!g.host) {
+    constexpr size_t bytes = (size_t)HOST_SLOT_RING * HOST_SLOT_WORDS * 8;
+    void* h = nullptr;
+    void* dev = nullptr;
+    if (hipHostMalloc(&h, bytes, hipHostMallocMapped | hipHostMallocCoherent) != hipSuccess || hipHostGetDevicePointer(&dev, h, 0) != hipSuccess || !dev) {
+      (void)hipGetLastError();
+      if (h) (void)hipHostFree(h);
+      g.failed = true;
+      return {};
+    }
+    std::memset(h, 0, bytes);
+    g.host = static_cast<uint64_t*>(h);
+    g.dev = static_cast<uint64_t*>(dev);
+  }
+  const uint64_t use = ++g.uses;
+  const size_t at = (size_t)host_slot_index(use) * HOST_SLOT_WORDS;
+  return HostSlot{g.dev + at, g.host + at, host_slot_seq(use)};
+}
+void host_slot_wait(const HostSlot& s, void* dst, size_t n) {
+  DFGPU_CHECK(s.dev && n <= (size_t)HOST_SLOT_PAYLOAD * 8, "internal: host slot read-back without a slot, or beyond its payload");
+  using clock = std::chrono::steady_clock;
+  hipStream_t stream = rt().stream;
+  const uint64_t* seq_word = const_cast<const uint64_t*>(s.host) + HOST_SLOT_SEQ;
+  const int64_t spin_us = option_int("runtime.host_slot_spin_us", HOST_SLOT_SPIN_US);
+  bool seen = __atomic_load_n(seq_word, __ATOMIC_ACQUIRE) == s.seq;
+  if (!seen && spin_us > 0) {
+    const auto t0 = clock::now();
+    const auto give_up = t0 + std::chrono::microseconds(spin_us);
+    auto next_query = t0 + std::chrono::microseconds(HOST_SLOT_QUERY_US);
+    for (;;) {
+      for (int i = 0; i < 32 && !seen; i++) {
+        cpu_pause();
+        seen = __atomic_load_n(seq_word, __ATOMIC_ACQUIRE) == s.seq;
+      }
+      if (seen) break;
+      const auto now = clock::now();
+      if (now >= next_query) {
+        const hipError_t e = hipStreamQuery(stream);
+        if (e == hipSuccess) break;
+        if (e != hipErrorNotReady) DFGPU_HIP(e);
+        (void)hipGetLastError();
+        next_query = now + std::chrono::microseconds(HOST_SLOT_QUERY_US);
+      }
+      if (now >= give_up) break;
+    }
+  }
+  if (!seen) {
+    DFGPU_HIP(hipStreamSynchronize(stream));
+    DFGPU_CHECK(__atomic_load_n(seq_word, __ATOMIC_ACQUIRE) == s.seq, "internal: the stream drained without the kernel's answer in its host slot");
+  }
+  std::memcpy(dst, const_cast<const uint64_t*>(s.host), n);
 }
 void h2d_async(void* dst, const void* src, size_t n) {
   DFGPU_HIP(hipMemcpyAsync(dst, src, n, hipMemcpyHostToDevice, rt().stream));
diff --git a/datafusion_amd/csrc/scan.hip b/datafusion_amd/csrc/scan.hip
--- a/datafusion_amd/csrc/scan.hip
+++ b/datafusion_amd/csrc/scan.hip
@@ -52,17 +52,21 @@
   if (threadIdx.x == 0) chunk_sums[blockIdx.x] = tot;
 }
 
-__global__ __launch_bounds__(BLOCK) void k_scan_sums(uint64_t* sums, int64_t n_chunks, uint64_t* total) {
-  uint64_t carry = 0;
+__global__ __launch_bounds__(BLOCK) void k_scan_sums(uint64_t* sums, int64_t n_chunks, uint64_t* total, uint64_t* slot, uint64_t slot_seq, const uint64_t* carry) {
+  uint64_t carry_sum = 0;
   for (int64_t base = 0; base < n_chunks; base += BLOCK) {
     int64_t i = base + threadIdx.x;
     uint64_t v = i < n_chunks ? sums[i] : 0;
     uint64_t tot;
     uint64_t ex = block_exclusive_scan(v, &tot);
-    if (i < n_chunks) sums[i] = carry + ex;
-    carry += tot;
+    if (i < n_chunks) sums[i] = carry_sum + ex;
+    carry_sum += tot;
   }
-  if (threadIdx.x == 0) *total = carry;
+  if (threadIdx.x == 0) {
+    *total = carry_sum;
+    const uint64_t answer[2] = {carry_sum, slot && carry ? *carry : 0};
+    host_slot_post(slot, slot_seq, answer, 2);
+  }
 }
 
 template <typename In>
@@ -87,7 +91,8 @@
 constexpr int CH_ITEMS = 16;
 constexpr int CH_CHUNK = BLOCK * CH_ITEMS;
 template <typename In>
-__global__ __launch_bounds__(BLOCK) void k_scan_chained(In in, int64_t n, uint64_t* __restrict__ state, unsigned* __restrict__ ticket, uint64_t* __restrict__ out) {
+__global__ __launch_bounds__(BLOCK) void k_scan_chained(In in, int64_t n, uint64_t* __restrict__ state, unsigned* __restrict__ ticket, uint64_t* __restrict__ out,
+                                                          uint64_t* slot, uint64_t slot_seq, const uint64_t* carry) {
   __shared__ unsigned s_tile;
   __shared__ uint64_t s_excl;
   if (threadIdx.x == 0) s_tile = atomicAdd(ticket, 1u);
@@ -108,7 +113,11 @@
     const uint64_t excl = lookback_exclusive(state, tile, tot);
     if (threadIdx.x == 0) {
       s_excl = excl;
-      if (tile == n_tiles - 1) out[n] = excl + tot;
+      if (tile == n_tiles - 1) {
+        out[n] = excl + tot;
+        const uint64_t answer[2] = {excl + tot, slot && carry ? *carry : 0};
+        host_slot_post(slot, slot_seq, answer, 2);
+      }
     }
   }
   __syncthreads();
@@ -121,18 +130,29 @@
 }
 
 template <typename In>
-static void run_scan(In in, int64_t n, uint64_t* out, const char* name) {
+static void run_scan(In in, int64_t n, uint64_t* out, const char* name, ScanTotal* total, const uint64_t* carry) {
   Runtime& r = rt();
+  if (total) {
+    *total = ScanTotal{};
+    total->carry = carry;
+  }
   if (n == 0) {
     DFGPU_HIP(hipMemsetAsync(out, 0, 8, r.stream));
+    if (total) total->known = !carry;
     return;
+  }
+  HostSlot slot;
+  if (total) {
+    slot = host_slot_acquire();
+    total->slot = slot;
+    total->dev_word = out + n;
   }
   const int64_t n_tiles_ch = (n + CH_CHUNK - 1) / CH_CHUNK;
   if (n_tiles_ch <= option_int("scan.chained_max_tiles", 8)) {
     const int64_t n_tiles = n_tiles_ch;
     BufPtr state = make_zero_buf((size_t)(n_tiles + 2) * 8);
     ProfileScope ps(name, 0);
-    k_scan_chained<<<(unsigned)n_tiles, BLOCK, 0, r.stream>>>(in, n, state->as<uint64_t>(), reinterpret_cast<unsigned*>(state->as<uint64_t>() + n_tiles), out);
+    k_scan_chained<<<(unsigned)n_tiles, BLOCK, 0, r.stream>>>(in, n, state->as<uint64_t>(), reinterpret_cast<unsigned*>(state->as<uint64_t>() + n_tiles), out, slot.dev, slot.seq, carry);
     DFGPU_HIP(hipGetLastError());
     return;
   }
@@ -140,15 +160,30 @@
   BufPtr sums = make_buf((size_t)n_chunks * 8);
   ProfileScope ps(name, 0);
   k_scan_reduce<<<(unsigned)n_chunks, BLOCK, 0, r.stream>>>(in, n, sums->as<uint64_t>());
-  k_scan_sums<<<1, BLOCK, 0, r.stream>>>(sums->as<uint64_t>(), n_chunks, out + n);
+  k_scan_sums<<<1, BLOCK, 0, r.stream>>>(sums->as<uint64_t>(), n_chunks, out + n, slot.dev, slot.seq, carry);
   k_scan_down<<<(unsigned)n_chunks, BLOCK, 0, r.stream>>>(in, n, sums->as<uint64_t>(), out);
   DFGPU_HIP(hipGetLastError());
 }
 
-void scan_mask_popcounts(const uint64_t* mask, const uint64_t* valid, int64_t nrows, uint64_t* out_prefix) {
+void scan_mask_popcounts(const uint64_t* mask, const uint64_t* valid, int64_t nrows, uint64_t* out_prefix, ScanTotal* total, const uint64_t* carry) {
   int64_t n_words = (nrows + 63) / 64;
-  run_scan(InMaskPopc{mask, valid, nrows}, n_words, out_prefix, "scan_mask_popcounts");
+  run_scan(InMaskPopc{mask, valid, nrows}, n_words, out_prefix, "scan_mask_popcounts", total, carry);
 }
-void scan_u32(const uint32_t* in, int64_t n, uint64_t* out_prefix) { run_scan(InU32{in}, n, out_prefix, "scan_u32"); }
+void scan_u32(const uint32_t* in, int64_t n, uint64_t* out_prefix, ScanTotal* total) { run_scan(InU32{in}, n, out_prefix, "scan_u32", total, nullptr); }
+
+uint64_t ScanTotal::get() {
+  if (known) return value;
+  if (slot) {
+    uint64_t answer[2] = {0, 0};
+    host_slot_wait(slot, answer, sizeof answer);
+    value = answer[0];
+    carried = answer[1];
+  } else {
+    value = dev_word ? read_u64(dev_word) : 0;
+    if (carry) d2h(&carried, carry, 8);
+  }
+  known = true;
+  return value;
+}
 
 }
diff --git a/datafusion_amd/csrc/sort.hip b/datafusion_amd/csrc/sort.hip
--- a/datafusion_amd/csrc/sort.hip
+++ b/datafusion_amd/csrc/sort.hip
@@ -1948,8 +1948,9 @@
 static BufPtr compact_mask(const BufPtr& mask, int64_t n, int64_t at_least, int64_t at_most, int64_t& m) {
   const int64_t n_words = (n + 63) / 64;
   BufPtr prefix = make_buf((size_t)(n_words + 1) * 8);
-  scan_mask_popcounts(mask->as<uint64_t>(), nullptr, n, prefix->as<uint64_t>());
-  m = (int64_t)read_u64(prefix->as<uint64_t>() + n_words);
+  ScanTotal scan_total;
+  scan_mask_popcounts(mask->as<uint64_t>(), nullptr, n, prefix->as<uint64_t>(), &scan_total);
+  m = (int64_t)scan_total.get();
   if (m < at_least || m > at_most) return nullptr;
   BufPtr ids = make_buf((size_t)(m ? m : 1) * 8);
   mask_to_ids(mask->as<uint64_t>(), prefix->as<uint64_t>(), n, m, ids->as<int64_t>());
```

After: 343.9 billion rows/s. No clear change (-0.6%).
